# Sewer56/dxt-lossless-transform

Measured on AMD Instinct MI355X. Metric: GiB/s BC blocks transformed (fwd+inv), higher is better.
Workload: dtype u8

## Files before the change

dxt-lossless-transform_amd/_build.py:

```python
from __future__ import annotations

import hashlib
import os
import shutil
import subprocess
from concurrent.futures import ThreadPoolExecutor

_HERE = os.path.dirname(os.path.abspath(__file__))
CSRC = os.path.join(_HERE, "csrc")
LIB_PATH = os.path.join(_HERE, "libdxtlt_gfx950.so")
_BUILD_DIR = os.path.join(os.path.dirname(_HERE), "build")

SOURCES = ["bcn_kernels.hip", "batch_kernels.hip", "dxtlt_api.cpp", "host_staging.cpp", "host_sharded.cpp", "c_api_core.cpp", "c_api_stable.cpp", "auto_transform.cpp", "file_format.cpp",
           "bc7_kernels.hip", "bc7_api.cpp", "bc6h_kernels.hip", "bc6h_api.cpp", "granule_launch.cpp", "granule_host.cpp", "bc1_normalize.hip", "normalize_api.cpp", "batch_api.cpp", "bc23_normalize.hip",
           "normalize23_api.cpp", "color565_ops.hip", "color565_api.cpp", "bcn_decode.hip", "decode_api.cpp",
           "auto_kernels.hip", "numa_affinity.cpp", "estimate_kernels.hip", "estimate_api.cpp", "batch_auto_kernels.hip", "batch_auto_api.cpp", "pixel_kernels.hip", "pixels_api.cpp",
           "image_kernels.hip", "image_regions_kernels.hip", "image_api.cpp", "image_batch_kernels.hip", "image_batch_api.cpp",
           "bc7_image_kernels.hip", "bc7_image_regions_kernels.hip", "bc7_image_api.cpp",
           "bc7_image_batch_kernels.hip", "bc7_image_batch_api.cpp",
           "bc6h_image_kernels.hip", "bc6h_image_regions_kernels.hip", "bc6h_image_api.cpp"]
BASE_FLAGS = ["--offload-arch=gfx950", "-O3", "-std=c++17", "-fPIC", "-Wall", "-Wextra", "-Wno-unused-command-line-argument"]


def _extra_flags(extra_flags=None) -> list:
    return list(extra_flags or [])


def _dirs(extra: list):
    if not extra:
        return os.path.join(_BUILD_DIR, "obj"), LIB_PATH
    tag = hashlib.sha256(" ".join(extra).encode()).hexdigest()[:12]
    side = os.path.join(_BUILD_DIR, "side-" + tag)
    return os.path.join(side, "obj"), os.path.join(side, "libdxtlt_gfx950.so")


def _hipcc() -> str:
    for cand in (os.environ.get("HIPCC"), shutil.which("hipcc"), "/opt/rocm/bin/hipcc"):
        if cand and os.path.exists(cand):
            return cand
    raise RuntimeError("hipcc not found: libdxtlt_gfx950.so cannot be built (set HIPCC)")


def _sources():
    return [os.path.join(CSRC, s) for s in SOURCES if os.path.exists(os.path.join(CSRC, s))]


def _headers():
    inc = os.path.join(os.path.dirname(_HERE), "include")
    files = [os.path.join(CSRC, f) for f in os.listdir(CSRC) if f.endswith(".h")]
    if os.path.isdir(inc):
        files += [os.path.join(inc, f) for f in os.listdir(inc) if f.endswith(".h")]
    return files


def is_stale() -> bool:
    if not os.path.exists(LIB_PATH):
        return True
    t = os.path.getmtime(LIB_PATH)
    return any(os.path.getmtime(f) > t for f in _sources() + _headers())


def build(force: bool = False, verbose: bool = False, extra_flags=None) -> str:
    extra = _extra_flags(extra_flags)
    obj_dir, lib_path = _dirs(extra)
    if not extra and not force and not is_stale():
        return LIB_PATH
    hipcc = _hipcc()
    os.makedirs(obj_dir, exist_ok=True)
    flags = BASE_FLAGS + extra
    newest_header = max((os.path.getmtime(h) for h in _headers()), default=0.0)

    def obj(src: str) -> str:
        return os.path.join(obj_dir, os.path.basename(src) + ".o")

    todo = []
    for src in _sources():
        o = obj(src)
        if force or not os.path.exists(o) or os.path.getmtime(o) < max(os.path.getmtime(src), newest_header):
            todo.append(src)

    def compile_one(src: str) -> None:
        cmd = [hipcc] + flags + ["-x", "hip", "-c", src, "-o", obj(src) + ".tmp"]
        if verbose:
            print(" ".join(cmd))
        subprocess.check_call(cmd)
        os.replace(obj(src) + ".tmp", obj(src))

    with ThreadPoolExecutor(max_workers=min(8, os.cpu_count() or 1)) as pool:
        list(pool.map(compile_one, todo))
    if not todo and os.path.exists(lib_path) and all(os.path.getmtime(obj(s)) <= os.path.getmtime(lib_path) for s in _sources()):
        return lib_path
    cmd = [hipcc, "--offload-arch=gfx950", "-shared", "-fPIC"] + [obj(s) for s in _sources()] + ["-o", lib_path + ".tmp", "-lpthread"]
    if verbose:
        print(" ".join(cmd))
    subprocess.check_call(cmd)
    os.replace(lib_path + ".tmp", lib_path)
    return lib_path


if __name__ == "__main__":
    print(build(force=True, verbose=True))
```

dxt-lossless-transform_amd/csrc/batch_api.cpp:

```cpp
#include <hip/hip_runtime_api.h>

#include <algorithm>
#include <condition_variable>
#include <cstdlib>
#include <cstring>
#include <exception>
#include <mutex>
#include <thread>
#include <vector>

#include "../../include/dxtlt_gfx950.h"
#include "bcn_launch.h"
#include "granule_launch.h"
#include "host_common.h"
#include "table_ring.h"

namespace {

using namespace dxtlt_host;
using dxtlt::BatchEntry;

inline uint32_t item_block_bytes(uint8_t format)
{
    return is_pixel_format(format) ? (uint32_t)pixel_bytes_of(format) : format == 1 || format == 4 ? 8u : 16u;
}

const char* const kDeviceFormatText = "batch item: format must be 1..5 (BC1..BC5), 6 (BC6H) or 7 (BC7; 6 and 7 are this build's own formats; "
                                      "pixel formats 8 and 9 go through dxtlt_transform_batch_host or the calls of dxtlt_pixels.h)";
const char* const kHostFormatText = "batch item: format must be 1..5 (BC1..BC5), 6 (BC6H), 7 (BC7), 8 (4-byte pixels) or 9 (3-byte pixels; "
                                    "6 to 9 are this build's own formats)";

inline bool pixel_item_overlaps(const DxtltBatchItem& it)
{
    if (!is_pixel_format(it.format) || it.len == 0)
        return false;
    const uintptr_t a = reinterpret_cast<uintptr_t>(it.d_input), b = reinterpret_cast<uintptr_t>(it.d_output);
    return a < b + it.len && b < a + it.len;
}

int32_t launch_pixel_item(const DxtltBatchItem& it, void* stream)
{
    const uint64_t pixels = it.len / item_block_bytes(it.format);
    return pixel_device_range(pixel_bytes_of(it.format), it.inverse != 0, it.d_input, it.d_output, pixels, 0, pixels,
                              pixel_decorrelate_of(it.decorrelation_mode),
                              pixel_layout_of(it.split_alpha_endpoints != 0, it.split_colour_endpoints != 0), stream);
}

thread_local dxtlt_host::TableRing g_ring;

const bool kTableByCopyEngine = dxtlt::experiment_env("DXTLT_BATCH_TABLE_COPY") != nullptr && dxtlt::experiment_env("DXTLT_BATCH_TABLE_COPY")[0] == '1';

}

dxtlt_host::TableRing& dxtlt_host::thread_table_ring() { return g_ring; }

hipError_t dxtlt_host::upload_table(TableSlot* slot, size_t bytes, hipStream_t stream)
{
    if (kTableByCopyEngine)
        return hipMemcpyAsync(slot->dev, slot->host, bytes, hipMemcpyHostToDevice, stream);
    return dxtlt::launch_table_upload(slot->host_mapped, slot->dev, bytes, stream);
}

namespace {

int32_t batch_device(const DxtltBatchItem* items, size_t count, void* hip_stream, bool pixels_allowed)
{
    if (count == 0)
        return kOk;
    if (items == nullptr)
        return fail(kInvalidArgument, "NULL item array with count > 0");
    for (size_t i = 0; i < count; ++i) {
        const DxtltBatchItem& it = items[i];
        if (it.format < 1 || it.format > (pixels_allowed ? 9 : 7))
            return fail(kInvalidArgument, kDeviceFormatText);
        if (it.len % item_block_bytes(it.format) != 0)
            return fail(kInvalidLength, "batch item: len is not a multiple of the block size");
        if (it.decorrelation_mode > 3 && dxtlt::format_has_colour(it.format))
            return fail(kInvalidArgument, "batch item: decorrelation_mode must be 0..3");
        if (it.len > 0 && (it.d_input == nullptr || it.d_output == nullptr))
            return fail(kInvalidArgument, "batch item: NULL device buffer with len > 0");
        if (pixel_item_overlaps(it))
            return fail(kInvalidArgument, "batch item: pixel input and output overlap");
    }
    for (const int format : {7, 6}) {
        uint64_t granules[2] = {0, 0};
        for (size_t i = 0; i < count; ++i)
            if (items[i].format == format)
                granules[items[i].inverse ? 1 : 0] += items[i].len / 16 / 1024;
        if (granules[0] > 0xFFFFFFull || granules[1] > 0xFFFFFFull)
            return fail(kInvalidArgument, dxtlt::granule::named(format, "batch too large for one launch (256 GiB or more of ", " in one direction)"));
    }
    hipStream_t user = static_cast<hipStream_t>(hip_stream);

    struct Group {
        std::vector<BatchEntry> entries;
        uint32_t wgs = 0;
        uint32_t uniform_wgs = 0;
        bool uniform = true;
    };
    constexpr int kGroups = 5 * 2 * 16;
    std::vector<Group> groups(kGroups);
    auto group_settings = [](int gi) {
        dxtlt::Settings s{};
        s.variant = (gi >> 2) & 3;
        s.split_alpha = ((gi >> 1) & 1) != 0;
        s.split_colour = (gi & 1) != 0;
        return s;
    };
    std::vector<size_t> singles;
    for (size_t i = 0; i < count; ++i) {
        const DxtltBatchItem& it = items[i];
        if (it.len == 0 || dxtlt::granule::is_granule_format(it.format) || is_pixel_format(it.format))
            continue;
        if (it.len >= (size_t(64) << 30))
            return fail(kInvalidArgument, "batch item of 64 GiB or more: use the single-buffer entry point");
        const bool colour = dxtlt::format_has_colour(it.format);
        const int sa = dxtlt::format_has_alpha_split(it.format) && it.split_alpha_endpoints ? 1 : 0;
        const int sc = colour && it.split_colour_endpoints ? 1 : 0, mode = colour ? it.decorrelation_mode : 0;
        const int gi = (((it.format - 1) * 2 + (it.inverse ? 1 : 0)) << 4) | (mode << 2) | (sa << 1) | sc;
        Group& g = groups[gi];
        BatchEntry e{};
        e.src = static_cast<const uint8_t*>(it.d_input);
        e.dst = static_cast<uint8_t*>(it.d_output);
        e.blocks = it.len / item_block_bytes(it.format);
        e.first_wg = g.wgs;
        const uint32_t wgs = dxtlt::plan_batch_entry((dxtlt::Format)it.format, it.inverse != 0, group_settings(gi), e);
        if (wgs == 0xFFFFFFFFu) {
            singles.push_back(i);
            continue;
        }
        if ((uint64_t)g.wgs + wgs > 0xFFFFFFull)
            return fail(kInvalidArgument, "batch too large for one launch (64 GiB or more of one format, direction and settings)");
        g.wgs += wgs;
        g.entries.push_back(e);
        if (g.entries.size() == 1)
            g.uniform_wgs = wgs;
        else if (wgs != g.uniform_wgs)
            g.uniform = false;
    }
    static const bool no_uniform = dxtlt::experiment_env("DXTLT_BATCH_NO_UNIFORM") != nullptr;
    static const bool no_strided = dxtlt::experiment_env("DXTLT_BATCH_NO_STRIDED") != nullptr;

    using GranuleEntry = dxtlt::granule::BatchEntry;
    struct GranulePlan {
        std::vector<GranuleEntry> entries, tails;
        std::vector<uint32_t> coarse;
        uint64_t wgs = 0;
        size_t at = 0, entry_bytes = 0, tail_bytes = 0, bytes = 0;
    };
    GranulePlan granule_plans[4];
    size_t table_bytes = 0;
    for (int q = 0; q < 4; ++q) {
        GranulePlan& p = granule_plans[q];
        const int inverse = q & 1, format = q < 2 ? 7 : 6;
        for (size_t i = 0; i < count; ++i) {
            const DxtltBatchItem& it = items[i];
            if (it.format != format || it.len == 0 || (it.inverse != 0) != (inverse != 0))
                continue;
            const uint64_t blocks = it.len / 16, tail = blocks % 1024, main = blocks - tail;
            const uint8_t* src = static_cast<const uint8_t*>(it.d_input);
            uint8_t* dst = static_cast<uint8_t*>(it.d_output);
            if (main != 0) {
                p.entries.push_back({src, dst, main, (uint32_t)p.wgs, 0});
                p.wgs += main / 1024;
            }
            if (tail != 0)
                p.tails.push_back({src + main * 16, dst + main * 16, 0, 0, (uint32_t)tail});
        }
        if (p.entries.empty() && p.tails.empty())
            continue;
        p.coarse.resize(((size_t)p.wgs + 63) / 64);
        size_t cur = 0;
        for (size_t k = 0; k < p.coarse.size(); ++k) {
            while (cur + 1 < p.entries.size() && p.entries[cur + 1].first_wg <= (uint32_t)(k * 64))
                ++cur;
            p.coarse[k] = (uint32_t)cur;
        }
        p.entry_bytes = p.entries.size() * sizeof(GranuleEntry);
        p.tail_bytes = p.tails.size() * sizeof(GranuleEntry);
        p.bytes = (p.entry_bytes + p.tail_bytes + p.coarse.size() * sizeof(uint32_t) + 15) & ~(size_t)15;
        p.at = table_bytes;
        table_bytes += p.bytes;
    }

    struct Placed {
        int gi;
        size_t at, entry_bytes;
    };
    std::vector<Placed> placed;
    for (int gi = 0; gi < kGroups; ++gi) {
        const Group& g = groups[gi];
        if (g.entries.empty())
            continue;
        const size_t entry_bytes = (g.entries.size() * sizeof(BatchEntry) + 15) & ~(size_t)15;
        placed.push_back({gi, table_bytes, entry_bytes});
        table_bytes += entry_bytes + dxtlt::batch_index_bytes(g.wgs);
    }
    if (table_bytes != 0) {
        TableSlot* slot = nullptr;
        hipError_t e = g_ring.acquire(table_bytes, &slot);
        if (e != hipSuccess)
            return fail(kDevice, "batch table staging", e);
        for (const GranulePlan& p : granule_plans) {
            if (p.bytes == 0)
                continue;
            uint8_t* h = static_cast<uint8_t*>(slot->host) + p.at;
            if (p.entry_bytes) std::memcpy(h, p.entries.data(), p.entry_bytes);
            if (p.tail_bytes) std::memcpy(h + p.entry_bytes, p.tails.data(), p.tail_bytes);
            if (!p.coarse.empty()) std::memcpy(h + p.entry_bytes + p.tail_bytes, p.coarse.data(), p.coarse.size() * sizeof(uint32_t));
        }
        std::vector<bool> wide(placed.size());
        for (size_t k = 0; k < placed.size(); ++k) {
            const Group& g = groups[placed[k].gi];
            uint8_t* h = static_cast<uint8_t*>(slot->host) + placed[k].at;
            std::memcpy(h, g.entries.data(), g.entries.size() * sizeof(BatchEntry));
            wide[k] = dxtlt::build_batch_index(g.entries.data(), g.entries.size(), g.wgs, h + placed[k].entry_bytes);
        }
        e = upload_table(slot, table_bytes, user);
        const char* what = "batch table copy / launch";
        for (int q = 0; q < 4 && e == hipSuccess; ++q) {
            const GranulePlan& p = granule_plans[q];
            const int inverse = q & 1, format = q < 2 ? 7 : 6;
            if (p.bytes == 0)
                continue;
            const uint8_t* d = static_cast<const uint8_t*>(slot->dev) + p.at;
            e = dxtlt::granule::launch_batch(format, inverse != 0, reinterpret_cast<const GranuleEntry*>(d),
                                             reinterpret_cast<const uint32_t*>(d + p.entry_bytes + p.tail_bytes), (uint32_t)p.entries.size(),
                                             (uint32_t)p.wgs, reinterpret_cast<const GranuleEntry*>(d + p.entry_bytes),
                                             (uint32_t)p.tails.size(), user);
            if (e != hipSuccess)
                what = format == 7 ? "BC7 batch table copy / launch" : "BC6H batch table copy / launch";
        }
        for (size_t k = 0; k < placed.size() && e == hipSuccess; ++k) {
            const int gi = placed[k].gi;
            Group& g = groups[gi];
            const size_t n = g.entries.size();
            const bool uniform = g.uniform && !no_uniform;
            bool strided = uniform && !no_strided;
            const int64_t src_stride = n >= 2 ? (int64_t)(g.entries[1].src - g.entries[0].src) : 0;
            const int64_t dst_stride = n >= 2 ? (int64_t)(g.entries[1].dst - g.entries[0].dst) : 0;
            for (size_t i = 1; i < n && strided; ++i) {
                const BatchEntry &a = g.entries[0], &b = g.entries[i];
                strided = b.blocks == a.blocks && b.full_tiles == a.full_tiles && b.form == a.form && b.halo_vecs == a.halo_vecs &&
                          std::memcmp(b.shift, a.shift, sizeof a.shift) == 0 && std::memcmp(b.gbase, a.gbase, sizeof a.gbase) == 0 &&
                          b.src == a.src + (int64_t)i * src_stride && b.dst == a.dst + (int64_t)i * dst_stride;
            }
            const uint8_t* d = static_cast<const uint8_t*>(slot->dev) + placed[k].at;
            e = dxtlt::launch_batch((dxtlt::Format)((gi >> 5) + 1), ((gi >> 4) & 1) != 0, group_settings(gi),
                                    reinterpret_cast<const BatchEntry*>(d), d + placed[k].entry_bytes, (uint32_t)n, g.wgs,
                                    uniform ? g.uniform_wgs : 0, wide[k], user, strided ? &g.entries[0] : nullptr, src_stride, dst_stride);
        }
        hipError_t ev = hipEventRecord(slot->done, user);
        slot->pending = ev == hipSuccess;
        if (e != hipSuccess)
            return fail(kDevice, what, e);
        if (ev != hipSuccess)
            return fail(kDevice, "batch event", ev);
    }
    for (size_t i : singles) {
        const DxtltBatchItem& it = items[i];
        dxtlt::Settings s{};
        s.variant = it.decorrelation_mode;
        s.split_alpha = it.split_alpha_endpoints != 0;
        s.split_colour = it.split_colour_endpoints != 0;
        s = dxtlt::effective_settings((dxtlt::Format)it.format, s);
        const uint64_t blocks = it.len / item_block_bytes(it.format);
        const hipError_t e = dxtlt::launch_transform((dxtlt::Format)it.format, it.inverse != 0, s, it.d_input, it.d_output,
                                                     dxtlt::Range{blocks, 0, blocks}, user);
        if (e != hipSuccess)
            return fail(kDevice, "batch item launch", e);
    }
    for (size_t i = 0; i < count; ++i)
        if (is_pixel_format(items[i].format) && items[i].len != 0)
            if (int32_t rc = launch_pixel_item(items[i], user); rc != kOk)
                return rc;
    return kOk;
}

}

extern "C" int32_t dxtlt_transform_batch_device(const DxtltBatchItem* items, size_t count, void* hip_stream)
{
    return batch_device(items, count, hip_stream, false);
}

extern "C" uint32_t dxtlt_debug_plan_batch(int32_t format, int32_t inverse, int32_t variant, int32_t split_alpha, int32_t split_colour,
                                           const uint64_t* src_addresses, const uint64_t* dst_addresses, const uint64_t* blocks, size_t count,
                                           DxtltDebugPlannedEntry* entries_out, uint8_t* index_out, size_t index_capacity,
                                           uint32_t* index_is_wide_out)
{
    if (index_is_wide_out)
        *index_is_wide_out = 0;
    if (format < 1 || format > 5 || (count != 0 && (!src_addresses || !dst_addresses || !blocks || !entries_out)))
        return 0xFFFFFFFFu;
    dxtlt::Settings s{};
    s.variant = variant;
    s.split_alpha = split_alpha != 0;
    s.split_colour = split_colour != 0;
    s = dxtlt::effective_settings((dxtlt::Format)format, s);
    std::vector<BatchEntry> entries;
    uint32_t total = 0;
    for (size_t i = 0; i < count; ++i) {
        BatchEntry e{};
        e.src = reinterpret_cast<const uint8_t*>(static_cast<uintptr_t>(src_addresses[i]));
        e.dst = reinterpret_cast<uint8_t*>(static_cast<uintptr_t>(dst_addresses[i]));
        e.blocks = blocks[i];
        e.first_wg = total;
        const uint32_t wgs = dxtlt::plan_batch_entry((dxtlt::Format)format, inverse != 0, s, e);
        if (wgs == 0xFFFFFFFFu || (uint64_t)total + wgs > 0xFFFFFFull)
            return 0xFFFFFFFFu;
        if (wgs == 0)
            e.end_wg = e.first_wg;
        total += wgs;
        DxtltDebugPlannedEntry& o = entries_out[i];
        o.first_wg = e.first_wg;
        o.end_wg = e.end_wg;
        o.full_tiles = e.full_tiles;
        o.form = e.form;
        o.halo_vecs = e.halo_vecs;
        std::memcpy(o.shift, e.shift, sizeof o.shift);
        std::memcpy(o.gbase, e.gbase, sizeof o.gbase);
        if (wgs != 0)
            entries.push_back(e);
    }
    if (total != 0) {
        if (index_out == nullptr || index_capacity < dxtlt::batch_index_bytes(total))
            return 0xFFFFFFFFu;
        const bool wide = dxtlt::build_batch_index(entries.data(), entries.size(), total, index_out);
        if (index_is_wide_out)
            *index_is_wide_out = wide ? 1 : 0;
    }
    return total;
}

namespace {

size_t env_number(const char* name, size_t fallback)
{
    const char* v = std::getenv(name);
    const unsigned long long x = v ? std::strtoull(v, nullptr, 10) : 0;
    return x ? (size_t)x : fallback;
}
const size_t kHostBatchChunkBytes = env_number("DXTLT_BATCH_CHUNK_MIB", 64) << 20;
const int kCopyThreads = (int)std::min<size_t>(64, env_number("DXTLT_BATCH_THREADS", 6));

struct PinnedArenas {
    void* in[2] = {nullptr, nullptr};
    void* out[2] = {nullptr, nullptr};
    size_t cap = 0;
    ~PinnedArenas() { release(); }
    void release()
    {
        for (int i = 0; i < 2; ++i) {
            if (in[i]) (void)hipHostFree(in[i]);
            if (out[i]) (void)hipHostFree(out[i]);
            in[i] = out[i] = nullptr;
        }
        cap = 0;
    }
    hipError_t reserve(size_t bytes)
    {
        if (bytes <= cap)
            return hipSuccess;
        release();
        for (int i = 0; i < 2; ++i) {
            hipError_t e = hipHostMalloc(&in[i], bytes, hipHostMallocDefault);
            if (e == hipSuccess)
                e = hipHostMalloc(&out[i], bytes, hipHostMallocDefault);
            if (e != hipSuccess) {
                release();
                return e;
            }
        }
        cap = bytes;
        return hipSuccess;
    }
};
thread_local PinnedArenas g_pinned;
#define g_pinned_in(c) (pinned_in[(c) & 1])
#define g_pinned_out(c) (pinned_out[(c) & 1])

struct HostBatchShared {
    std::mutex m;
    std::condition_variable cv;
    std::vector<int> packed;
    std::vector<int> unpacked;
    int uploaded_recorded = 0;
    int kernels_issued = 0;
    int enqueued = 0;
    bool failed = false;
    hipError_t error = hipSuccess;
};

}

void dxtlt_host::release_batch_thread_tables()
{
    g_ring.release();
    g_pinned.release();
}

extern "C" int32_t dxtlt_transform_batch_host(const DxtltBatchItem* items, size_t count)
{
    if (count == 0)
        return kOk;
    if (items == nullptr)
        return fail(kInvalidArgument, "NULL item array with count > 0");
    uint64_t total = 0;
    for (size_t i = 0; i < count; ++i) {
        const DxtltBatchItem& it = items[i];
        if (it.format < 1 || it.format > 9)
            return fail(kInvalidArgument, kHostFormatText);
        if (it.len % item_block_bytes(it.format) != 0)
            return fail(kInvalidLength, "batch item: len is not a multiple of the block size");
        if (it.decorrelation_mode > 3 && dxtlt::format_has_colour(it.format))
            return fail(kInvalidArgument, "batch item: decorrelation_mode must be 0..3");
        if (it.len > 0 && (it.d_input == nullptr || it.d_output == nullptr))
            return fail(kInvalidArgument, "batch item: NULL buffer with len > 0");
        if (pixel_item_overlaps(it))
            return fail(kInvalidArgument, "batch item: pixel input and output overlap");
        if (it.len >= (size_t(4) << 30))
            return fail(kInvalidArgument, "batch item of 4 GiB or more: use the single-buffer entry point");
        total += (it.len + 255) & ~uint64_t(255);
    }
    if (total == 0)
        return kOk;

    const uint64_t big_item = 2 * (uint64_t)kHostBatchChunkBytes;
    std::vector<DxtltBatchItem> small;
    small.reserve(count);
    for (size_t i = 0; i < count; ++i) {
        const DxtltBatchItem& it = items[i];
        if (it.len < big_item) {
            small.push_back(it);
            continue;
        }
        int32_t rc;
        if (is_pixel_format(it.format))
            rc = pixel_host_call(pixel_bytes_of(it.format), it.inverse != 0, static_cast<const uint8_t*>(it.d_input),
                                 static_cast<uint8_t*>(it.d_output), it.len, pixel_decorrelate_of(it.decorrelation_mode),
                                 pixel_layout_of(it.split_alpha_endpoints != 0, it.split_colour_endpoints != 0));
        else if (dxtlt::granule::is_granule_format(it.format))
            rc = dxtlt_host::granule_host_call(it.format, it.inverse != 0, static_cast<const uint8_t*>(it.d_input),
                                               static_cast<uint8_t*>(it.d_output), it.len);
        else
            rc = dxtlt_host::transform(it.format, it.inverse != 0, static_cast<const uint8_t*>(it.d_input),
                                       static_cast<uint8_t*>(it.d_output), it.len, it.decorrelation_mode,
                                       dxtlt::format_has_alpha_split(it.format) && it.split_alpha_endpoints, it.split_colour_endpoints != 0);
        if (rc != kOk)
            return rc;
    }
    if (small.empty())
        return kOk;
    items = small.data();
    count = small.size();

    std::vector<uint64_t> slot(count);
    std::vector<size_t> chunk_first;
    std::vector<uint64_t> chunk_bytes;
    {
        uint64_t in_chunk = 0;
        chunk_first.push_back(0);
        for (size_t i = 0; i < count; ++i) {
            const uint64_t padded = (items[i].len + 255) & ~uint64_t(255);
            if (in_chunk > 0 && in_chunk + padded > kHostBatchChunkBytes) {
                chunk_first.push_back(i);
                chunk_bytes.push_back(in_chunk);
                in_chunk = 0;
            }
            slot[i] = in_chunk;
            in_chunk += padded;
        }
        chunk_first.push_back(count);
        chunk_bytes.push_back(in_chunk);
    }
    const int nchunks = (int)chunk_bytes.size();
    const uint64_t arena_bytes = *std::max_element(chunk_bytes.begin(), chunk_bytes.end());

    void *d_in = nullptr, *d_out = nullptr;
    hipStream_t up = nullptr;
    if (int32_t rc = acquire_staging((size_t)(2 * arena_bytes), &d_in, &d_out, &up); rc != kOk)
        return rc;
    if (hipError_t e = g_pinned.reserve((size_t)arena_bytes); e != hipSuccess)
        return fail(kDevice, "hipHostMalloc(batch arenas)", e);
    void* const pinned_in[2] = {g_pinned.in[0], g_pinned.in[1]};
    void* const pinned_out[2] = {g_pinned.out[0], g_pinned.out[1]};
    int dev = 0;
    (void)hipGetDevice(&dev);
    hipStream_t down = nullptr;
    if (hipError_t e = hipStreamCreateWithFlags(&down, hipStreamNonBlocking); e != hipSuccess)
        return fail(kDevice, "hipStreamCreate(download)", e);

    std::vector<hipEvent_t> ev((size_t)nchunks * 3, nullptr);
    for (auto& e : ev)
        if (hipError_t err = hipEventCreateWithFlags(&e, hipEventDisableTiming); err != hipSuccess) {
            for (auto& e2 : ev) if (e2) (void)hipEventDestroy(e2);
            (void)hipStreamDestroy(down);
            return fail(kDevice, "hipEventCreate", err);
        }
    auto ev_uploaded = [&](int c) { return ev[(size_t)c * 3]; };
    auto ev_kernels = [&](int c) { return ev[(size_t)c * 3 + 1]; };
    auto ev_downloaded = [&](int c) { return ev[(size_t)c * 3 + 2]; };

    HostBatchShared sh;
    sh.packed.assign((size_t)nchunks, 0);
    sh.unpacked.assign((size_t)nchunks, 0);
    auto set_failed = [&](hipError_t e) {
        std::lock_guard<std::mutex> lk(sh.m);
        if (!sh.failed) {
            sh.failed = true;
            sh.error = e;
        }
        sh.cv.notify_all();
    };

    auto packer = [&](int tid) {
        hipError_t e = hipSetDevice(dev);
        for (int c = 0; c < nchunks && e == hipSuccess; ++c) {
            if (c < 2) {
                std::lock_guard<std::mutex> lk(sh.m);
                if (sh.failed)
                    return;
            }
            if (c >= 2) {
                {
                    std::unique_lock<std::mutex> lk(sh.m);
                    sh.cv.wait(lk, [&] { return sh.uploaded_recorded > c - 2 || sh.failed; });
                    if (sh.failed)
                        return;
                }
                e = hipEventSynchronize(ev_uploaded(c - 2));
                if (e != hipSuccess)
                    break;
            }
            uint8_t* arena = static_cast<uint8_t*>(g_pinned_in(c));
            for (size_t i = chunk_first[(size_t)c] + (size_t)tid; i < chunk_first[(size_t)c + 1]; i += kCopyThreads)
                if (items[i].len)
                    std::memcpy(arena + slot[i], items[i].d_input, items[i].len);
            {
                std::lock_guard<std::mutex> lk(sh.m);
                sh.packed[(size_t)c]++;
            }
            sh.cv.notify_all();
        }
        if (e != hipSuccess)
            set_failed(e);
    };
    auto unpacker = [&](int tid) {
        hipError_t e = hipSetDevice(dev);
        for (int c = 0; c < nchunks && e == hipSuccess; ++c) {
            {
                std::unique_lock<std::mutex> lk(sh.m);
                sh.cv.wait(lk, [&] { return sh.enqueued > c || sh.failed; });
                if (sh.enqueued <= c)
                    return;
            }
            e = hipEventSynchronize(ev_downloaded(c));
            if (e != hipSuccess)
                break;
            const uint8_t* arena = static_cast<const uint8_t*>(g_pinned_out(c));
            for (size_t i = chunk_first[(size_t)c] + (size_t)tid; i < chunk_first[(size_t)c + 1]; i += kCopyThreads)
                if (items[i].len)
                    std::memcpy(items[i].d_output, arena + slot[i], items[i].len);
            {
                std::lock_guard<std::mutex> lk(sh.m);
                sh.unpacked[(size_t)c]++;
            }
            sh.cv.notify_all();
        }
        if (e != hipSuccess)
            set_failed(e);
    };

    std::vector<std::thread> threads;
    bool spawn_failed = false;
    auto spawn = [&](auto&& fn, auto... args) {
        if (spawn_failed)
            return;
        try {
            threads.emplace_back(fn, args...);
        } catch (const std::exception&) {
            spawn_failed = true;
        }
    };
    for (int t = 0; t < kCopyThreads; ++t) spawn(packer, t);
    for (int t = 0; t < kCopyThreads; ++t) spawn(unpacker, t);

    auto downloader = [&] {
        hipError_t e = hipSetDevice(dev);
        for (int c = 0; c < nchunks && e == hipSuccess; ++c) {
            {
                std::unique_lock<std::mutex> lk(sh.m);
                sh.cv.wait(lk, [&] { return (sh.kernels_issued > c && (c < 2 || sh.unpacked[(size_t)c - 2] == kCopyThreads)) || sh.failed; });
                if (sh.failed)
                    return;
            }
            const uint8_t* dout = static_cast<const uint8_t*>(d_out) + (size_t)(c & 1) * arena_bytes;
            e = hipStreamWaitEvent(down, ev_kernels(c), 0);
            if (e == hipSuccess)
                e = hipMemcpyAsync(g_pinned_out(c), dout, (size_t)chunk_bytes[(size_t)c], hipMemcpyDeviceToHost, down);
            if (e == hipSuccess)
                e = hipEventRecord(ev_downloaded(c), down);
            if (e != hipSuccess)
                break;
            {
                std::lock_guard<std::mutex> lk(sh.m);
                sh.enqueued = c + 1;
            }
            sh.cv.notify_all();
        }
        if (e != hipSuccess)
            set_failed(e);
    };
    spawn(downloader);
    if (spawn_failed) {
        set_failed(hipErrorOutOfMemory);
        for (auto& t : threads)
            t.join();
        for (auto& e : ev) (void)hipEventDestroy(e);
        (void)hipStreamDestroy(down);
        return fail(kAllocation, "could not start the batch copy threads");
    }

    int32_t rc = kOk;
    hipError_t err = hipSuccess;
    std::vector<DxtltBatchItem> dev_items;
    for (int c = 0; c < nchunks && rc == kOk && err == hipSuccess; ++c) {
        {
            std::unique_lock<std::mutex> lk(sh.m);
            sh.cv.wait(lk, [&] { return (sh.packed[(size_t)c] == kCopyThreads && (c < 2 || sh.enqueued > c - 2)) || sh.failed; });
            if (sh.failed)
                break;
        }
        uint8_t* di = static_cast<uint8_t*>(d_in) + (size_t)(c & 1) * arena_bytes;
        uint8_t* dout = static_cast<uint8_t*>(d_out) + (size_t)(c & 1) * arena_bytes;
        if (c >= 2)
            err = hipStreamWaitEvent(up, ev_kernels(c - 2), 0);
        if (err == hipSuccess)
            err = hipMemcpyAsync(di, g_pinned_in(c), (size_t)chunk_bytes[(size_t)c], hipMemcpyHostToDevice, up);
        if (err == hipSuccess)
            err = hipEventRecord(ev_uploaded(c), up);
        {
            std::lock_guard<std::mutex> lk(sh.m);
            if (err == hipSuccess)
                sh.uploaded_recorded = c + 1;
        }
        sh.cv.notify_all();
        if (err != hipSuccess)
            break;
        if (c >= 2)
            err = hipStreamWaitEvent(up, ev_downloaded(c - 2), 0);
        if (err != hipSuccess)
            break;
        dev_items.clear();
        for (size_t i = chunk_first[(size_t)c]; i < chunk_first[(size_t)c + 1]; ++i) {
            DxtltBatchItem it = items[i];
            it.d_input = di + slot[i];
            it.d_output = dout + slot[i];
            dev_items.push_back(it);
        }
        rc = batch_device(dev_items.data(), dev_items.size(), up, true);
        if (rc != kOk)
            break;
        err = hipEventRecord(ev_kernels(c), up);
        if (err != hipSuccess)
            break;
        {
            std::lock_guard<std::mutex> lk(sh.m);
            sh.kernels_issued = c + 1;
        }
        sh.cv.notify_all();
    }
    if (rc != kOk || err != hipSuccess) {
        std::lock_guard<std::mutex> lk(sh.m);
        sh.failed = true;
        if (err != hipSuccess && sh.error == hipSuccess)
            sh.error = err;
        sh.cv.notify_all();
    }
    for (auto& t : threads)
        t.join();
    (void)hipStreamSynchronize(up);
    (void)hipStreamSynchronize(down);
    for (auto& e : ev) (void)hipEventDestroy(e);
    (void)hipStreamDestroy(down);
    if (rc != kOk)
        return rc;
    if (sh.failed)
        return fail(kDevice, "host batch copy", sh.error);
    return kOk;
}
```

dxt-lossless-transform_amd/csrc/batch_kernels.hip:

```cpp
#include <cstdlib>
#include <cstring>
#include <vector>

#include "bcn_device.h"

#include "batch_lookup.h"

namespace dxtlt {

struct BatchView {
    const uint8_t* src;
    uint8_t* dst;
    uint64_t blocks;
    uint32_t first_wg, end_wg, full_tiles;
    uint32_t flags;
    uint32_t shifts[2];
    uint64_t gbase[6];
};

__device__ __forceinline__ BatchView load_batch_entry(const BatchEntry* entry)
{
    const uint64_t* q = reinterpret_cast<const uint64_t*>(entry);
    const uint32_t* w = reinterpret_cast<const uint32_t*>(entry);
    BatchView v;
    v.src = (const uint8_t*)(global_cptr)q[0];
    v.dst = (uint8_t*)(global_ptr)q[1];
    v.blocks = q[2];
    v.first_wg = w[6];
    v.end_wg = w[7];
    v.full_tiles = w[8];
    v.flags = w[9];
    v.shifts[0] = w[10];
    v.shifts[1] = w[11];
#pragma unroll
    for (int i = 0; i < 6; ++i)
        v.gbase[i] = q[6 + i];
    return v;
}
__device__ __forceinline__ void pin_batch_view(BatchView& v)
{
#ifdef DXTLT_WG_TIMING
    (void)v;
    return;
#endif
    uint64_t s = reinterpret_cast<uintptr_t>(v.src), d = reinterpret_cast<uintptr_t>(v.dst);
    asm("" : "+s"(s), "+s"(d), "+s"(v.blocks));
    v.src = (const uint8_t*)(global_cptr)s;
    v.dst = (uint8_t*)(global_ptr)d;
    asm("" : "+s"(v.first_wg), "+s"(v.end_wg), "+s"(v.full_tiles), "+s"(v.flags), "+s"(v.shifts[0]), "+s"(v.shifts[1]));
#pragma unroll
    for (int i = 0; i < 6; ++i)
        asm("" : "+s"(v.gbase[i]));
}
static_assert(offsetof(BatchEntry, first_wg) == 24 && offsetof(BatchEntry, end_wg) == 28 && offsetof(BatchEntry, full_tiles) == 32 && offsetof(BatchEntry, form) == 36 &&
                  offsetof(BatchEntry, shift) == 40 && offsetof(BatchEntry, gbase) == 48,
              "load_batch_entry reads BatchEntry by dword offsets");

constexpr uint32_t kBatchAligned = 1;

struct StridedBatch {
    BatchEntry first;
    int64_t src_stride, dst_stride;
    uint32_t on;
};

#ifdef DXTLT_WG_TIMING
__device__ uint32_t g_wg_timing[4 << 20];
extern "C" int dxtlt_debug_read_wg_timing(uint32_t* out, size_t count)
{
    return (int)hipMemcpyFromSymbol(out, HIP_SYMBOL(g_wg_timing), count * 4);
}
extern "C" int dxtlt_debug_read_wg_marks(uint32_t* out, size_t count)
{
    return (int)hipMemcpyFromSymbol(out, HIP_SYMBOL(dxtlt::g_wg_marks), count * 4);
}
#define WG_TIMING_BEGIN const uint64_t t_begin = __builtin_amdgcn_s_memrealtime();
#define WG_TIMING_END(kind)                                                                         \
    do {                                                                                            \
        __builtin_amdgcn_s_waitcnt(0);                                                              \
        asm volatile("s_waitcnt vmcnt(0)" ::: "memory");                                            \
        if (threadIdx.x == 0 && blockIdx.x < (1u << 20)) {                                          \
            uint32_t xcc;                                                                           \
            asm volatile("s_getreg_b32 %0, hwreg(HW_REG_XCC_ID)" : "=s"(xcc));                       \
            g_wg_timing[4 * blockIdx.x] = (uint32_t)(__builtin_amdgcn_s_memrealtime() - t_begin);   \
            g_wg_timing[4 * blockIdx.x + 1] = (kind);                                               \
            g_wg_timing[4 * blockIdx.x + 2] = (uint32_t)t_begin;                                    \
            g_wg_timing[4 * blockIdx.x + 3] = xcc & 0xF;                                            \
        }                                                                                           \
    } while (0)
#else
#define WG_TIMING_BEGIN
#define WG_TIMING_END(kind)
#endif

template <int FMT, int VARIANT, bool SA, bool SC, bool INVERSE, int THREADS = batch_tile_threads(FMT, SC, INVERSE)>
__global__ void __launch_bounds__(THREADS)
batch_kernel(const BatchEntry* __restrict__ entries_arg, const uint8_t* __restrict__ index_arg, uint32_t n_base, uint32_t uniform_wgs,
             uint32_t magic, StridedBatch strided)
{
    constexpr int kLds = INVERSE ? shift_lds_bytes(1, THREADS) : halo_lds_bytes<FMT, THREADS>();
    __shared__ __attribute__((aligned(16))) uint8_t lds[kLds];
    const uint32_t wg = blockIdx.x;
    WG_TIMING_BEGIN
    BatchView en;
    uint32_t e;
    uint64_t entries_at = reinterpret_cast<uintptr_t>(entries_arg), index_at = reinterpret_cast<uintptr_t>(index_arg);
#ifndef DXTLT_WG_TIMING
    asm("" : "+s"(entries_at), "+s"(index_at), "+s"(n_base), "+s"(uniform_wgs), "+s"(magic));
#endif
    const BatchEntry* entries = (const BatchEntry*)(const __attribute__((address_space(1))) BatchEntry*)entries_at;
    const uint8_t* index = (const uint8_t*)(global_cptr)index_at;
    if (uniform_wgs != 0) {
        e = __umulhi(wg, magic);
        if ((e + 1) * uniform_wgs <= wg)
            ++e;
        if (strided.on != 0) {
            const BatchEntry& f = strided.first;
            en.src = (const uint8_t*)(global_cptr)(reinterpret_cast<uintptr_t>(f.src) + (uint64_t)((int64_t)e * strided.src_stride));
            en.dst = (uint8_t*)(global_ptr)(reinterpret_cast<uintptr_t>(f.dst) + (uint64_t)((int64_t)e * strided.dst_stride));
            en.blocks = f.blocks;
            en.first_wg = e * uniform_wgs;
            en.end_wg = en.first_wg + uniform_wgs;
            en.full_tiles = f.full_tiles;
            en.flags = (uint32_t)f.form | ((uint32_t)f.halo_vecs << 8) | ((uint32_t)f.natural << 16);
            en.shifts[0] = (uint32_t)f.shift[0] | ((uint32_t)f.shift[1] << 8) | ((uint32_t)f.shift[2] << 16) | ((uint32_t)f.shift[3] << 24);
            en.shifts[1] = (uint32_t)f.shift[4] | ((uint32_t)f.shift[5] << 8);
#pragma unroll
            for (int i = 0; i < 6; ++i)
                en.gbase[i] = f.gbase[i];
        } else {
            en = load_batch_entry(entries + e);
        }
    } else {
        e = batch_entry_of_workgroup(entries, index, n_base, magic, wg, en);
    }
    const uint32_t n_wgs = en.end_wg - en.first_wg;
    uint32_t local = wg - en.first_wg;
    if (n_wgs >= 8) {
        local += (en.first_wg + n_wgs - 1u - e) & 7u;
        local = local >= n_wgs ? local - n_wgs : local;
    }
    const bool aligned = (en.flags & 0xFF) == kBatchAligned;
    if (aligned && local < en.full_tiles) {
        if constexpr (INVERSE)
            inv_aligned_tile<FMT, VARIANT, SA, SC, THREADS>(en.src, en.dst, en.blocks, 0, local, lds);
        else
            fwd_aligned_tile<FMT, VARIANT, SA, SC, THREADS>(en.src, en.dst, en.blocks, 0, local, lds);
        WG_TIMING_END(1);
        return;
    }
    Shifts sh;
#pragma unroll
    for (int i = 0; i < 6; ++i) {
        sh.d[i] = (int)((en.shifts[i >> 2] >> (8 * (i & 3))) & 127u);
        sh.gbase[i] = en.gbase[i];
    }
#ifdef DXTLT_EXPERIMENTS
    sh.xcd_remap = 0;
    sh.line_policy = INVERSE ? 1 : 3;
    sh.skip_partial = 0;
#endif
    sh.natural = 1;
    sh.halo_vecs = (int)(en.flags >> 8) & 0xFF;
    sh.full_tiles = en.full_tiles;
    sh.range_blocks = en.blocks;
    if constexpr (INVERSE) {
        if (local < en.full_tiles) {
            const uint64_t tile = xcd_contiguous_tile(local, en.full_tiles);
            inv_shift_tile<FMT, VARIANT, SA, SC, THREADS>(en.src, en.dst, en.blocks, 0, sh, tile, lds);
            WG_TIMING_END(2);
            return;
        }
        inv_shift_edge_tile<FMT, VARIANT, SA, SC, THREADS>(en.src, en.dst, en.blocks, sh, en.full_tiles, lds);
        WG_TIMING_END(4);
    } else {
        if (local != 0 && local < en.full_tiles) {
            fwd_halo_tile<FMT, VARIANT, SA, SC, kNormNone, true, THREADS>(en.src, en.dst, en.blocks, 0, sh, local, lds);
            WG_TIMING_END(2);
            return;
        }
        fwd_halo_edge_tile<FMT, VARIANT, SA, SC, kNormNone, true, THREADS>(en.src, en.dst, sh, local, lds);
        WG_TIMING_END(local == 0 ? 3 : 4);
    }
}

uint32_t plan_batch_entry(Format fmt, bool inverse, const Settings& s, BatchEntry& e)
{
    if (e.blocks == 0)
        return 0;
    const Settings es = effective_settings(fmt, s);
    const Streams S = make_streams(fmt, es.split_alpha, es.split_colour);
    const void* soa = inverse ? (const void*)e.src : (const void*)e.dst;
    const uint64_t T = (uint64_t)tile_blocks(fmt, batch_tile_threads(fmt, es.split_colour, inverse));
    const uint64_t tiles = e.blocks / T, rest = e.blocks % T;
    const uint64_t mask = inverse ? 15 : (uint64_t)(kHaloAlign - 1);
    bool on_lines = true, stream_tails = false;
    int d[6] = {0, 0, 0, 0, 0, 0}, halo_blocks = 0;
    for (int i = 0; i < S.n; ++i) {
        const uint64_t base = reinterpret_cast<uintptr_t>(soa) + (uint64_t)S.off[i] * e.blocks;
        d[i] = (int)(base & mask);
        on_lines = on_lines && (base & 127) == 0;
        stream_tails = stream_tails || d[i] != 0;
        halo_blocks = std::max(halo_blocks, (d[i] + S.width[i] - 1) / S.width[i]);
    }
    if (!shifts_are_natural(S, d))
        return 0xFFFFFFFFu;
    e.form = on_lines ? 1 : 0;
    e.natural = 1;
    e.reserved = 0;
    e.reserved2[0] = e.reserved2[1] = 0;
    const int per_vec = 16 / fmt_block(fmt);
    e.halo_vecs = inverse ? 0 : (uint8_t)((halo_blocks + per_vec - 1) / per_vec);
    for (int i = 0; i < 6; ++i) {
        e.shift[i] = (uint8_t)d[i];
        e.gbase[i] = i < S.n ? (uint64_t)S.off[i] * e.blocks - (uint64_t)d[i] : 0;
    }
    e.full_tiles = (uint32_t)tiles;
    const bool edge = rest != 0 || (!inverse && stream_tails);
    const uint32_t wgs = (uint32_t)tiles + (edge ? 1u : 0u);
    e.end_wg = e.first_wg + wgs;
    return wgs;
}

bool build_batch_index(const BatchEntry* entries, size_t n_entries, uint32_t total_wgs, uint8_t* index)
{
    const size_t n_base = batch_index_base_count(total_wgs), n_delta = batch_index_delta_count(total_wgs);
    uint32_t* base = reinterpret_cast<uint32_t*>(index);
    std::memset(index, 0, batch_index_bytes(total_wgs));
    std::vector<uint32_t> d(n_delta);
    uint32_t largest = 0;
    size_t cur = 0;
    for (size_t j = 0; j < n_delta; ++j) {
        const uint32_t wg = (uint32_t)(j * kBatchIndexWgs);
        while (cur + 1 < n_entries && entries[cur].end_wg <= wg)
            ++cur;
        if (wg % kBatchBaseWgs == 0)
            base[wg / kBatchBaseWgs] = (uint32_t)cur;
        d[j] = (uint32_t)(cur - base[wg / kBatchBaseWgs]);
        largest = std::max(largest, d[j]);
    }
    const bool wide = largest > 255;
    uint8_t* delta = index + n_base * 4;
    for (size_t j = 0; j < n_delta; ++j) {
        if (wide) {
            delta[2 * j] = (uint8_t)d[j];
            delta[2 * j + 1] = (uint8_t)(d[j] >> 8);
        } else {
            delta[j] = (uint8_t)d[j];
        }
    }
    return wide;
}

namespace {

using BatchFn = void (*)(const BatchEntry*, const uint8_t*, uint32_t, uint32_t, uint32_t, StridedBatch);

template <int FMT, int VARIANT, bool SA, bool SC>
BatchFn batch_fn(bool inverse) { return inverse ? batch_kernel<FMT, VARIANT, SA, SC, true> : batch_kernel<FMT, VARIANT, SA, SC, false>; }

template <int FMT, int VARIANT>
BatchFn batch_splits(bool sa, bool sc, bool inverse)
{
    if constexpr (FMT == kBc3) {
        if (sa)
            return sc ? batch_fn<FMT, VARIANT, true, true>(inverse) : batch_fn<FMT, VARIANT, true, false>(inverse);
    }
    return sc ? batch_fn<FMT, VARIANT, false, true>(inverse) : batch_fn<FMT, VARIANT, false, false>(inverse);
}

template <int FMT>
BatchFn batch_bc45(bool split_endpoints, bool inverse)
{
    return split_endpoints ? batch_fn<FMT, kNone, true, false>(inverse) : batch_fn<FMT, kNone, false, false>(inverse);
}

template <int FMT>
BatchFn batch_variant(int variant, bool sa, bool sc, bool inverse)
{
    switch (variant) {
    case kNone: return batch_splits<FMT, kNone>(sa, sc, inverse);
    case kVar1: return batch_splits<FMT, kVar1>(sa, sc, inverse);
    case kVar2: return batch_splits<FMT, kVar2>(sa, sc, inverse);
    default: return batch_splits<FMT, kVar3>(sa, sc, inverse);
    }
}

}

hipError_t launch_batch(Format fmt, bool inverse, const Settings& s, const BatchEntry* d_entries, const uint8_t* d_index,
                        uint32_t n_entries, uint32_t total_wgs, uint32_t uniform_wgs, bool wide_index, hipStream_t stream,
                        const BatchEntry* strided_first, int64_t src_stride, int64_t dst_stride)
{
    if (n_entries == 0 || total_wgs == 0)
        return hipSuccess;
    if (s.variant < 0 || s.variant > 3 || total_wgs > 0xFFFFFFu)
        return hipErrorInvalidValue;
    if (uniform_wgs != 0 && (uint64_t)uniform_wgs * n_entries != total_wgs)
        return hipErrorInvalidValue;
    const uint32_t magic = uniform_wgs > 1 ? (uint32_t)((1ull << 32) / uniform_wgs) : uniform_wgs == 1 ? 0xFFFFFFFFu : n_entries;
    static const bool no_array = experiment_env("DXTLT_BATCH_NO_ARRAY") != nullptr;
    if (strided_first != nullptr && uniform_wgs != 0 && !no_array && strided_first->form == 1) {
        const hipError_t e = launch_tiled_array(fmt, inverse, s, strided_first->src, strided_first->dst, strided_first->blocks, n_entries,
                                                src_stride, dst_stride, stream);
        if (e != hipErrorNotSupported)
            return e;
    }
    StridedBatch strided{};
    if (strided_first != nullptr && uniform_wgs != 0) {
        strided.first = *strided_first;
        strided.src_stride = src_stride;
        strided.dst_stride = dst_stride;
        strided.on = 1;
    }
    const Settings es = effective_settings(fmt, s);
    const bool sa = es.split_alpha, sc = es.split_colour;
    BatchFn k = nullptr;
    switch (fmt) {
    case kBc1: k = batch_variant<kBc1>(es.variant, false, sc, inverse); break;
    case kBc2: k = batch_variant<kBc2>(es.variant, false, sc, inverse); break;
    case kBc3: k = batch_variant<kBc3>(es.variant, sa, sc, inverse); break;
    case kBc4: k = batch_bc45<kBc4>(sa, inverse); break;
    case kBc5: k = batch_bc45<kBc5>(sa, inverse); break;
    default: return hipErrorInvalidValue;
    }
    hipLaunchKernelGGL(k, dim3(total_wgs), dim3(batch_tile_threads(fmt, sc, inverse)), 0, stream, d_entries, d_index,
                       (uint32_t)batch_index_base_count(total_wgs) | (wide_index ? 0x80000000u : 0u), uniform_wgs, magic, strided);
    return hipGetLastError();
}

}
```

dxt-lossless-transform_amd/csrc/bcn_device.h:

```cpp
#pragma once
#include <hip/hip_runtime.h>

#include <algorithm>
#include <cstddef>
#include <type_traits>

#include "bc1_normalize.h"
#include "bcn_launch.h"
#include "streaming_store.h"
#include "ycocg_swar.h"

namespace dxtlt {

typedef uint32_t u32x4 __attribute__((ext_vector_type(4)));
typedef uint32_t u32x2 __attribute__((ext_vector_type(2)));

constexpr int kThreads = 256;
constexpr int default_tile_threads(int fmt, bool inverse)
{
    (void)inverse;
    return fmt == kBc1 || fmt == kBc4 ? 128 : 256;
}

#ifndef DXTLT_NONTEMPORAL
#define DXTLT_NONTEMPORAL 1
#endif

#ifdef DXTLT_WG_TIMING
__device__ uint32_t g_wg_marks[8 << 20];
__device__ __forceinline__ void wg_mark(int i)
{
    if (threadIdx.x == 0 && blockIdx.x < (1u << 20))
        g_wg_marks[8 * blockIdx.x + i] = (uint32_t)__builtin_amdgcn_s_memrealtime();
}
#define WG_MARK(i) wg_mark(i)
#define WG_MARK_LOADS_DONE(i)                                  \
    do {                                                       \
        asm volatile("s_waitcnt vmcnt(0)" ::: "memory");       \
        wg_mark(i);                                            \
    } while (0)
#else
#define WG_MARK(i)
#define WG_MARK_LOADS_DONE(i)
#endif

__device__ __forceinline__ u32x4 gload16(const void* p)
{
#if DXTLT_NONTEMPORAL
    return __builtin_nontemporal_load(reinterpret_cast<const u32x4*>(p));
#else
    return *reinterpret_cast<const u32x4*>(p);
#endif
}

__device__ __forceinline__ void gstore16(void* p, u32x4 v)
{
#if DXTLT_NONTEMPORAL
    store_streaming16(p, v);
#else
    *reinterpret_cast<u32x4*>(p) = v;
#endif
}

__device__ __forceinline__ void gstore16_aos(uint8_t* aos_base, void* p, u32x4 v)
{
    if ((reinterpret_cast<uintptr_t>(aos_base) & 15) == 0)
        gstore16(p, v);
    else
        __builtin_nontemporal_store(v, reinterpret_cast<u32x4*>(p));
}

template <int I, int N, typename F>
__device__ __forceinline__ void static_for(F&& f)
{
    if constexpr (I < N) {
        f(std::integral_constant<int, I>{});
        static_for<I + 1, N>(f);
    }
}

template <int W, int WAVES, typename F>
__device__ __forceinline__ void for_this_wave_from(int w, F&& f)
{
    if constexpr (W + 1 >= WAVES) {
        f(std::integral_constant<int, W>{});
    } else {
        if (w == W)
            f(std::integral_constant<int, W>{});
        else
            for_this_wave_from<W + 1, WAVES>(w, f);
    }
}
template <int WAVES, typename F>
__device__ __forceinline__ void for_this_wave(int t, F&& f)
{
    for_this_wave_from<0, WAVES>(__builtin_amdgcn_readfirstlane(t >> 6), f);
}

__host__ __device__ constexpr int fmt_block(int fmt) { return fmt == kBc1 || fmt == kBc4 ? 8 : 16; }
__host__ __device__ constexpr int tile_blocks(int fmt, int threads) { return threads * 16 / fmt_block(fmt); }

template <int FMT, bool SA, bool SC, int T>
__device__ __forceinline__ uint64_t soa_offset_of_image_byte(int o, uint64_t total_blocks, uint64_t blk0)
{
    constexpr Streams S = make_streams(FMT, SA, SC);
    uint64_t r = 0;
#pragma unroll
    for (int s = 0; s < S.n; ++s) {
        const int lo = S.off[s] * T;
        const int hi = lo + S.width[s] * T;
        if (o >= lo && o < hi)
            r = (uint64_t)S.off[s] * total_blocks + (uint64_t)S.width[s] * blk0 + (uint64_t)(o - lo);
    }
    return r;
}

#ifndef DXTLT_WAVE_OFFSETS
#define DXTLT_WAVE_OFFSETS 1
#endif
template <int FMT, bool SA, bool SC, int T, int W>
__device__ __forceinline__ uint64_t soa_offset_of_image_byte_in_wave(int o, uint64_t total_blocks, uint64_t blk0)
{
    constexpr Streams S = make_streams(FMT, SA, SC);
    constexpr int wave_lo = W * 1024, wave_hi = wave_lo + 1024;
    uint64_t r = 0;
    static_for<0, S.n>([&](auto si) {
        constexpr int s = decltype(si)::value;
        constexpr int lo = S.off[s] * T;
        constexpr int hi = lo + S.width[s] * T;
        if constexpr (lo < wave_hi && hi > wave_lo) {
            constexpr bool only = lo <= wave_lo && hi >= wave_hi;
            const uint64_t base = (uint64_t)S.off[s] * total_blocks + (uint64_t)S.width[s] * blk0;
            if (only || (o >= lo && o < hi))
                r = base + (uint64_t)(uint32_t)(o - lo);
        }
    });
    return r;
}

template <int FMT, bool SA, bool SC, int THREADS>
__device__ __forceinline__ uint64_t soa_offset_of_lane(int t, uint64_t total_blocks, uint64_t blk0)
{
    constexpr int T = tile_blocks(FMT, THREADS);
#if DXTLT_WAVE_OFFSETS
    uint64_t o = 0;
    for_this_wave<THREADS / 64>(t, [&](auto wi) {
        o = soa_offset_of_image_byte_in_wave<FMT, SA, SC, T, decltype(wi)::value>(t * 16, total_blocks, blk0);
    });
    return o;
#else
    return soa_offset_of_image_byte<FMT, SA, SC, T>(t * 16, total_blocks, blk0);
#endif
}

template <typename T>
__device__ __forceinline__ T& lds_at(uint8_t* lds, int byte_off)
{
    return *reinterpret_cast<T*>(lds + byte_off);
}

typedef volatile uint16_t __attribute__((address_space(3))) lds_halfword;
__device__ __forceinline__ lds_halfword* lds_halfwords(uint8_t* lds, int byte_off)
{
    return (lds_halfword*)(lds + byte_off);
}

#ifndef DXTLT_BC3_RECORD6
#define DXTLT_BC3_RECORD6 1
#endif
typedef uint32_t u32x2_align4 __attribute__((ext_vector_type(2), aligned(4)));
typedef volatile uint32_t __attribute__((address_space(3))) lds_dword;

__device__ __forceinline__ void lds_put_record6(uint8_t* lds, int addr, uint32_t lo16, uint32_t hi32)
{
#if DXTLT_BC3_RECORD6
    const bool odd = (addr & 2) != 0;
    const int a32 = odd ? addr + 2 : addr;
    const int a16 = odd ? addr : addr + 4;
    const uint32_t v32 = odd ? hi32 : (lo16 & 0xFFFFu) | (hi32 << 16);
    const uint32_t v16 = odd ? lo16 : hi32 >> 16;
    *(lds_dword*)(lds + a32) = v32;
    *lds_halfwords(lds, a16) = (uint16_t)v16;
#else
    lds_halfwords(lds, addr)[0] = (uint16_t)lo16;
    lds_halfwords(lds, addr)[1] = (uint16_t)hi32;
    lds_halfwords(lds, addr)[2] = (uint16_t)(hi32 >> 16);
#endif
}

__device__ __forceinline__ void lds_get_record6(uint8_t* lds, int addr, uint32_t& lo16, uint32_t& hi32)
{
#if DXTLT_BC3_RECORD6
    const u32x2_align4 w = *reinterpret_cast<const u32x2_align4*>(lds + (addr & ~3));
    const uint32_t sh = (uint32_t)(addr & 2) * 8u;
    const uint32_t rec = __builtin_amdgcn_alignbit(w.y, w.x, sh);
    lo16 = rec & 0xFFFFu;
    hi32 = (rec >> 16) | ((w.y >> sh) << 16);
#else
    lo16 = lds_at<uint16_t>(lds, addr + 0);
    hi32 = (uint32_t)lds_at<uint16_t>(lds, addr + 2) | ((uint32_t)lds_at<uint16_t>(lds, addr + 4) << 16);
#endif
}

template <bool SA, int T, int E>
__device__ __forceinline__ void scatter_bc4_half(uint8_t* lds, int b, uint32_t lo, uint32_t hi)
{
    if constexpr (SA) {
        lds_at<uint8_t>(lds, E * T + b) = (uint8_t)lo;
        lds_at<uint8_t>(lds, (E + 1) * T + b) = (uint8_t)(lo >> 8);
    } else {
        lds_at<uint16_t>(lds, E * T + 2 * b) = (uint16_t)lo;
    }
    lds_put_record6(lds, (E + 2) * T + 6 * b, lo >> 16, hi);
}

template <bool SA, int T, int E>
__device__ __forceinline__ void gather_bc4_half(uint8_t* lds, int b, uint32_t& lo, uint32_t& hi)
{
    uint32_t a01;
    if constexpr (SA)
        a01 = (uint32_t)lds_at<uint8_t>(lds, E * T + b) | ((uint32_t)lds_at<uint8_t>(lds, (E + 1) * T + b) << 8);
    else
        a01 = lds_at<uint16_t>(lds, E * T + 2 * b);
    uint32_t i01;
    lds_get_record6(lds, (E + 2) * T + 6 * b, i01, hi);
    lo = a01 | (i01 << 16);
}

template <int FMT, int VARIANT, bool SA, bool SC, int T>
__device__ __forceinline__ void scatter_to_image(uint8_t* lds, int u, u32x4 q)
{
    if constexpr (FMT == kBc4) {
        if constexpr (SA) {
            lds_at<uint16_t>(lds, 0 * T + 2 * u) = (uint16_t)((q.x & 0xFFu) | ((q.z & 0xFFu) << 8));
            lds_at<uint16_t>(lds, 1 * T + 2 * u) = (uint16_t)(((q.x >> 8) & 0xFFu) | (q.z & 0xFF00u));
        } else {
            lds_at<uint32_t>(lds, 0 * T + 4 * u) = (q.x & 0xFFFFu) | (q.z << 16);
        }
        lds_at<uint32_t>(lds, 2 * T + 12 * u + 0) = (q.x >> 16) | (q.y << 16);
        lds_at<uint32_t>(lds, 2 * T + 12 * u + 4) = (q.y >> 16) | (q.z & 0xFFFF0000u);
        lds_at<uint32_t>(lds, 2 * T + 12 * u + 8) = q.w;
    } else if constexpr (FMT == kBc5) {
        scatter_bc4_half<SA, T, 0>(lds, u, q.x, q.y);
        scatter_bc4_half<SA, T, 8>(lds, u, q.z, q.w);
    } else if constexpr (FMT == kBc1) {
        const uint32_t ca = decorrelate2<VARIANT>(q.x);
        const uint32_t cb = decorrelate2<VARIANT>(q.z);
        if constexpr (SC) {
            lds_at<uint32_t>(lds, 0 * T + 4 * u) = (ca & 0xFFFFu) | (cb << 16);
            lds_at<uint32_t>(lds, 2 * T + 4 * u) = (ca >> 16) | (cb & 0xFFFF0000u);
        } else {
            lds_at<u32x2>(lds, 0 * T + 8 * u) = u32x2{ca, cb};
        }
        lds_at<u32x2>(lds, 4 * T + 8 * u) = u32x2{q.y, q.w};
    } else if constexpr (FMT == kBc2) {
        const uint32_t c = decorrelate2<VARIANT>(q.z);
        lds_at<u32x2>(lds, 0 * T + 8 * u) = u32x2{q.x, q.y};
        if constexpr (SC) {
            lds_at<uint16_t>(lds, 8 * T + 2 * u) = (uint16_t)c;
            lds_at<uint16_t>(lds, 10 * T + 2 * u) = (uint16_t)(c >> 16);
        } else {
            lds_at<uint32_t>(lds, 8 * T + 4 * u) = c;
        }
        lds_at<uint32_t>(lds, 12 * T + 4 * u) = q.w;
    } else {
        const uint32_t c = decorrelate2<VARIANT>(q.z);
        if constexpr (SA) {
            lds_at<uint8_t>(lds, 0 * T + u) = (uint8_t)q.x;
            lds_at<uint8_t>(lds, 1 * T + u) = (uint8_t)(q.x >> 8);
        } else {
            lds_at<uint16_t>(lds, 0 * T + 2 * u) = (uint16_t)q.x;
        }
        lds_put_record6(lds, 2 * T + 6 * u, q.x >> 16, q.y);
        if constexpr (SC) {
            lds_at<uint16_t>(lds, 8 * T + 2 * u) = (uint16_t)c;
            lds_at<uint16_t>(lds, 10 * T + 2 * u) = (uint16_t)(c >> 16);
        } else {
            lds_at<uint32_t>(lds, 8 * T + 4 * u) = c;
        }
        lds_at<uint32_t>(lds, 12 * T + 4 * u) = q.w;
    }
}

template <int FMT, int VARIANT, bool SA, bool SC, int T>
__device__ __forceinline__ u32x4 gather_from_image(uint8_t* lds, int u)
{
    u32x4 q;
    if constexpr (FMT == kBc4) {
        uint32_t e;
        if constexpr (SA) {
            const uint32_t a0 = lds_at<uint16_t>(lds, 0 * T + 2 * u), a1 = lds_at<uint16_t>(lds, 1 * T + 2 * u);
            e = (a0 & 0xFFu) | ((a1 & 0xFFu) << 8) | ((a0 & 0xFF00u) << 8) | ((a1 & 0xFF00u) << 16);
        } else {
            e = lds_at<uint32_t>(lds, 0 * T + 4 * u);
        }
        const uint32_t r0 = lds_at<uint32_t>(lds, 2 * T + 12 * u + 0);
        const uint32_t r1 = lds_at<uint32_t>(lds, 2 * T + 12 * u + 4);
        const uint32_t r2 = lds_at<uint32_t>(lds, 2 * T + 12 * u + 8);
        q.x = (e & 0xFFFFu) | (r0 << 16);
        q.y = (r0 >> 16) | (r1 << 16);
        q.z = (e >> 16) | (r1 & 0xFFFF0000u);
        q.w = r2;
    } else if constexpr (FMT == kBc5) {
        uint32_t rlo, rhi, glo, ghi;
        gather_bc4_half<SA, T, 0>(lds, u, rlo, rhi);
        gather_bc4_half<SA, T, 8>(lds, u, glo, ghi);
        q = u32x4{rlo, rhi, glo, ghi};
    } else if constexpr (FMT == kBc1) {
        uint32_t ca, cb;
        if constexpr (SC) {
            const uint32_t c0 = lds_at<uint32_t>(lds, 0 * T + 4 * u);
            const uint32_t c1 = lds_at<uint32_t>(lds, 2 * T + 4 * u);
            ca = (c0 & 0xFFFFu) | (c1 << 16);
            cb = (c0 >> 16) | (c1 & 0xFFFF0000u);
        } else {
            const u32x2 p = lds_at<u32x2>(lds, 0 * T + 8 * u);
            ca = p.x;
            cb = p.y;
        }
        const u32x2 idx = lds_at<u32x2>(lds, 4 * T + 8 * u);
        q.x = recorrelate2<VARIANT>(ca);
        q.y = idx.x;
        q.z = recorrelate2<VARIANT>(cb);
        q.w = idx.y;
    } else if constexpr (FMT == kBc2) {
        const u32x2 a = lds_at<u32x2>(lds, 0 * T + 8 * u);
        uint32_t c;
        if constexpr (SC)
            c = (uint32_t)lds_at<uint16_t>(lds, 8 * T + 2 * u) | ((uint32_t)lds_at<uint16_t>(lds, 10 * T + 2 * u) << 16);
        else
            c = lds_at<uint32_t>(lds, 8 * T + 4 * u);
        q.x = a.x;
        q.y = a.y;
        q.z = recorrelate2<VARIANT>(c);
        q.w = lds_at<uint32_t>(lds, 12 * T + 4 * u);
    } else {
        uint32_t a01;
        if constexpr (SA)
            a01 = (uint32_t)lds_at<uint8_t>(lds, 0 * T + u) | ((uint32_t)lds_at<uint8_t>(lds, 1 * T + u) << 8);
        else
            a01 = lds_at<uint16_t>(lds, 0 * T + 2 * u);
        uint32_t i01, i2345;
        lds_get_record6(lds, 2 * T + 6 * u, i01, i2345);
        uint32_t c;
        if constexpr (SC)
            c = (uint32_t)lds_at<uint16_t>(lds, 8 * T + 2 * u) | ((uint32_t)lds_at<uint16_t>(lds, 10 * T + 2 * u) << 16);
        else
            c = lds_at<uint32_t>(lds, 8 * T + 4 * u);
        q.x = a01 | (i01 << 16);
        q.y = i2345;
        q.z = recorrelate2<VARIANT>(c);
        q.w = lds_at<uint32_t>(lds, 12 * T + 4 * u);
    }
    return q;
}

__device__ __forceinline__ uint64_t xcd_contiguous_tile(uint32_t orig, uint32_t nwg)
{
    const uint32_t q = nwg >> 3, r = nwg & 7, xcd = orig & 7;
    const uint32_t start = xcd < r ? xcd * (q + 1) : r * (q + 1) + (xcd - r) * q;
    return start + (orig >> 3);
}


template <int FMT, int NORM>
__device__ __forceinline__ u32x4 normalize_vector(u32x4 q)
{
    if constexpr (FMT == kBc1 && NORM != kNormNone) {
        uint32_t ca = q.x, xa = q.y, cb = q.z, xb = q.w;
        normalize_bc1_block<NORM>(ca, xa);
        normalize_bc1_block<NORM>(cb, xb);
        q = u32x4{ca, xa, cb, xb};
    }
    return q;
}

constexpr int kTiledArray = 2;

template <int FMT, int VARIANT, bool SA, bool SC, int THREADS, int NORM = kNormNone>
__device__ __forceinline__ void fwd_aligned_tile(const uint8_t* __restrict__ aos, uint8_t* __restrict__ soa,
                                                 uint64_t total_blocks, uint64_t first_block, uint64_t tile, uint8_t* lds)
{
    constexpr int T = tile_blocks(FMT, THREADS);
    const int t = threadIdx.x;
    WG_MARK(1);
    const u32x4 q = normalize_vector<FMT, NORM>(gload16(aos + tile * (THREADS * 16) + t * 16));
    WG_MARK_LOADS_DONE(2);
    scatter_to_image<FMT, VARIANT, SA, SC, T>(lds, t, q);
    __syncthreads();
    WG_MARK(3);
    const u32x4 v = lds_at<u32x4>(lds, t * 16);
    const uint64_t o = soa_offset_of_lane<FMT, SA, SC, THREADS>(t, total_blocks, first_block + tile * T);
    gstore16(soa + o, v);
    WG_MARK(4);
}

struct AosSink {
    template <int FMT, int THREADS>
    __device__ __forceinline__ void store(uint8_t* aos, uint64_t tile, int t, u32x4 q) const
    {
        gstore16_aos(aos, aos + tile * (THREADS * 16) + t * 16, q);
    }
    template <int FMT, int THREADS>
    __device__ __forceinline__ void store_edge(uint8_t* aos, uint64_t tile, int t, u32x4 q, int own) const
    {
        constexpr int PV = 16 / fmt_block(FMT);
        uint8_t* out = aos + tile * (THREADS * 16) + t * 16;
        if ((t + 1) * PV <= own)
            __builtin_nontemporal_store(q, reinterpret_cast<u32x4*>(out));
        else
            __builtin_nontemporal_store(u32x2{q.x, q.y}, reinterpret_cast<u32x2*>(out));
    }
};

template <int FMT, int VARIANT, bool SA, bool SC, int THREADS, typename SINK = AosSink>
__device__ __forceinline__ void inv_aligned_tile(const uint8_t* __restrict__ soa, uint8_t* __restrict__ aos,
                                                 uint64_t total_blocks, uint64_t first_block, uint64_t tile, uint8_t* lds,
                                                 const SINK& sink = SINK{})
{
    constexpr int T = tile_blocks(FMT, THREADS);
    const int t = threadIdx.x;
    const uint64_t o = soa_offset_of_lane<FMT, SA, SC, THREADS>(t, total_blocks, first_block + tile * T);
    lds_at<u32x4>(lds, t * 16) = gload16(soa + o);
    __syncthreads();
    const u32x4 q = gather_from_image<FMT, VARIANT, SA, SC, T>(lds, t);
    sink.template store<FMT, THREADS>(aos, tile, t, q);
}

template <int FMT, int VARIANT, bool SA, bool SC, int THREADS, int NORM = kNormNone>
__global__ void __launch_bounds__(THREADS)
fwd_tiled(const uint8_t* __restrict__ aos, uint8_t* __restrict__ soa, uint64_t total_blocks, uint64_t first_block,
          int xcd_remap, int64_t aos_stride, int64_t soa_stride)
{
    __shared__ __attribute__((aligned(16))) uint8_t lds[THREADS * 16];
    WG_MARK(0);
    if (xcd_remap & kTiledArray) {
        aos += (int64_t)blockIdx.y * aos_stride;
        soa += (int64_t)blockIdx.y * soa_stride;
    }
#ifdef DXTLT_EXPERIMENTS
    const uint64_t tile = (xcd_remap & 1) ? xcd_contiguous_tile(blockIdx.x, gridDim.x) : (uint64_t)blockIdx.x;
#else
    const uint64_t tile = blockIdx.x;
#endif
    fwd_aligned_tile<FMT, VARIANT, SA, SC, THREADS, NORM>(aos, soa, total_blocks, first_block, tile, lds);
}

template <int FMT, int VARIANT, bool SA, bool SC, int THREADS>
__global__ void __launch_bounds__(THREADS)
inv_tiled(const uint8_t* __restrict__ soa, uint8_t* __restrict__ aos, uint64_t total_blocks, uint64_t first_block,
          int xcd_remap, int64_t soa_stride, int64_t aos_stride)
{
    __shared__ __attribute__((aligned(16))) uint8_t lds[THREADS * 16];
    if (xcd_remap & kTiledArray) {
        soa += (int64_t)blockIdx.y * soa_stride;
        aos += (int64_t)blockIdx.y * aos_stride;
    }
#ifdef DXTLT_EXPERIMENTS
    const uint64_t tile = (xcd_remap & 1) ? xcd_contiguous_tile(blockIdx.x, gridDim.x) : (uint64_t)blockIdx.x;
#else
    const uint64_t tile = blockIdx.x;
#endif
    inv_aligned_tile<FMT, VARIANT, SA, SC, THREADS>(soa, aos, total_blocks, first_block, tile, lds);
}

struct Shifts {
    int d[6];
    int natural;
    int halo_vecs;
    uint64_t gbase[6];
    uint32_t full_tiles;
    uint64_t range_blocks;
#ifdef DXTLT_EXPERIMENTS
    int xcd_remap;
    int line_policy;
    int skip_partial;
#endif
};

__device__ __forceinline__ bool shifts_xcd_contiguous(const Shifts& sh, bool product_default)
{
#ifdef DXTLT_EXPERIMENTS
    (void)product_default;
    return sh.xcd_remap != 0;
#else
    (void)sh;
    return product_default;
#endif
}
__device__ __forceinline__ bool shifts_halo_write_through(const Shifts& sh)
{
#ifdef DXTLT_EXPERIMENTS
    return sh.line_policy == 3;
#else
    (void)sh;
    return true;
#endif
}
__device__ __forceinline__ bool shifts_skip_partial(const Shifts& sh)
{
#ifdef DXTLT_EXPERIMENTS
    return sh.skip_partial != 0;
#else
    (void)sh;
    return false;
#endif
}

template <typename STREAMS>
__host__ __device__ inline void fill_gbase(Shifts& sh, const STREAMS& S, uint64_t total_blocks, uint64_t first_block)
{
    for (int i = 0; i < 6; ++i)
        sh.gbase[i] = i < S.n ? (uint64_t)S.off[i] * total_blocks + (uint64_t)S.width[i] * first_block - (uint64_t)sh.d[i] : 0;
}

typedef const __attribute__((address_space(1))) uint8_t* global_cptr;
typedef __attribute__((address_space(1))) uint8_t* global_ptr;

__device__ __forceinline__ const uint8_t* fetched_now(const uint8_t* p)
{
    uint64_t v = reinterpret_cast<uintptr_t>(p);
    asm("" : "+s"(v));
    return (const uint8_t*)(global_cptr)v;
}
__device__ __forceinline__ uint8_t* fetched_now(uint8_t* p)
{
    uint64_t v = reinterpret_cast<uintptr_t>(p);
    asm("" : "+s"(v));
    return (uint8_t*)(global_ptr)v;
}

__device__ __forceinline__ Shifts shifts_fetched_at_once(const Shifts& in)
{
    Shifts s = in;
#ifdef DXTLT_EXPERIMENTS
    asm("" : "+s"(s.d[0]), "+s"(s.d[1]), "+s"(s.d[2]), "+s"(s.d[3]), "+s"(s.d[4]), "+s"(s.d[5]), "+s"(s.gbase[0]), "+s"(s.gbase[1]),
             "+s"(s.gbase[2]), "+s"(s.gbase[3]), "+s"(s.gbase[4]), "+s"(s.gbase[5]), "+s"(s.xcd_remap), "+s"(s.line_policy),
             "+s"(s.skip_partial), "+s"(s.natural), "+s"(s.halo_vecs), "+s"(s.full_tiles), "+s"(s.range_blocks));
#else
    asm("" : "+s"(s.d[0]), "+s"(s.d[1]), "+s"(s.d[2]), "+s"(s.d[3]), "+s"(s.d[4]), "+s"(s.d[5]), "+s"(s.gbase[0]), "+s"(s.gbase[1]),
             "+s"(s.gbase[2]), "+s"(s.gbase[3]), "+s"(s.gbase[4]), "+s"(s.gbase[5]), "+s"(s.natural), "+s"(s.halo_vecs),
             "+s"(s.full_tiles), "+s"(s.range_blocks));
#endif
    return s;
}

__host__ __device__ constexpr int stream_element_width(int bytes_per_block) { return bytes_per_block == 6 ? 2 : bytes_per_block; }

template <typename STREAMS>
__host__ __device__ inline int shifts_are_natural(const STREAMS& S, const int (&d)[6])
{
    int ok = 1;
    for (int i = 0; i < 6; ++i)
        if (i < S.n && (d[i] & (stream_element_width(S.width[i]) - 1)) != 0)
            ok = 0;
    return ok;
}


template <typename T>
using lds_volatile = volatile T __attribute__((address_space(3)));

template <int SIZE>
__device__ __forceinline__ void lds_put_piece(uint8_t* lds, int addr, uint64_t v)
{
    if constexpr (SIZE == 1) *(lds_volatile<uint8_t>*)(lds + addr) = (uint8_t)v;
    if constexpr (SIZE == 2) *(lds_volatile<uint16_t>*)(lds + addr) = (uint16_t)v;
    if constexpr (SIZE == 4) *(lds_volatile<uint32_t>*)(lds + addr) = (uint32_t)v;
    if constexpr (SIZE == 8) *(lds_volatile<uint64_t>*)(lds + addr) = v;
}

template <int SIZE>
__device__ __forceinline__ uint64_t lds_get_piece(uint8_t* lds, int addr)
{
    if constexpr (SIZE == 1) return *(lds_volatile<uint8_t>*)(lds + addr);
    if constexpr (SIZE == 2) return *(lds_volatile<uint16_t>*)(lds + addr);
    if constexpr (SIZE == 4) return *(lds_volatile<uint32_t>*)(lds + addr);
    if constexpr (SIZE == 8) return *(lds_volatile<uint64_t>*)(lds + addr);
    return 0;
}

constexpr int lds_piece_size(int W, int K, int P)
{
    const int a = K + P;
    int align = a == 0 ? W : (a & -a);
    if (align > W) align = W;
    int size = 1;
    while (size * 2 <= align && size * 2 <= W - P) size *= 2;
    return size;
}

template <int W, int K, int P = 0>
__device__ __forceinline__ void lds_put_seq(uint8_t* lds, int addr, uint64_t v)
{
    if constexpr (P < W) {
        constexpr int size = lds_piece_size(W, K, P);
        lds_put_piece<size>(lds, addr + P, v >> (8 * P));
        lds_put_seq<W, K, P + size>(lds, addr, v);
    }
}

template <int W, int K, int P = 0>
__device__ __forceinline__ uint64_t lds_get_seq(uint8_t* lds, int addr)
{
    if constexpr (P < W) {
        constexpr int size = lds_piece_size(W, K, P);
        return (lds_get_piece<size>(lds, addr + P) << (8 * P)) | lds_get_seq<W, K, P + size>(lds, addr);
    }
    return 0;
}

template <int W, bool NAT = false>
__device__ __forceinline__ void lds_put(uint8_t* lds, int addr, uint64_t v)
{
    if constexpr (W == 1 || NAT) {
        lds_put_piece<W>(lds, addr, v);
    } else {
        switch (addr & (W - 1)) {
        case 0: lds_put_seq<W, 0>(lds, addr, v); break;
        case 1: lds_put_seq<W, 1>(lds, addr, v); break;
        case 2: if constexpr (W > 2) lds_put_seq<W, 2>(lds, addr, v); break;
        case 3: if constexpr (W > 2) lds_put_seq<W, 3>(lds, addr, v); break;
        case 4: if constexpr (W > 4) lds_put_seq<W, 4>(lds, addr, v); break;
        case 5: if constexpr (W > 4) lds_put_seq<W, 5>(lds, addr, v); break;
        case 6: if constexpr (W > 4) lds_put_seq<W, 6>(lds, addr, v); break;
        default: if constexpr (W > 4) lds_put_seq<W, 7>(lds, addr, v); break;
        }
    }
}

template <int W, bool NAT = false>
__device__ __forceinline__ uint64_t lds_get(uint8_t* lds, int addr)
{
    if constexpr (W == 1 || NAT) {
        return lds_get_piece<W>(lds, addr);
    } else {
        switch (addr & (W - 1)) {
        case 0: return lds_get_seq<W, 0>(lds, addr);
        case 1: return lds_get_seq<W, 1>(lds, addr);
        case 2: if constexpr (W > 2) return lds_get_seq<W, 2>(lds, addr); break;
        case 3: if constexpr (W > 2) return lds_get_seq<W, 3>(lds, addr); break;
        case 4: if constexpr (W > 4) return lds_get_seq<W, 4>(lds, addr); break;
        case 5: if constexpr (W > 4) return lds_get_seq<W, 5>(lds, addr); break;
        case 6: if constexpr (W > 4) return lds_get_seq<W, 6>(lds, addr); break;
        default: if constexpr (W > 4) return lds_get_seq<W, 7>(lds, addr); break;
        }
        return 0;
    }
}

template <int FMT, bool SA, bool SC>
struct FieldStreams {
    static constexpr int alpha = 0;
    static constexpr int a1 = 1;
    static constexpr int aidx = SA ? 2 : 1;
    static constexpr int col = FMT == kBc1 ? 0 : FMT == kBc2 ? 1 : (SA ? 3 : 2);
    static constexpr int c1 = col + 1;
    static constexpr int idx = col + (SC ? 2 : 1);
    static constexpr int galpha = aidx + 1;
    static constexpr int ga1 = galpha + 1;
    static constexpr int gaidx = SA ? galpha + 2 : galpha + 1;
};

template <bool SA, bool NAT, int ALPHA, int A1, int AIDX>
__device__ __forceinline__ void scatter_shifted_bc4_block(uint8_t* lds, int b, uint32_t lo, uint32_t hi, const int (&base)[6])
{
    if constexpr (SA) {
        lds_put<1>(lds, base[ALPHA] + b, lo & 0xFF);
        lds_put<1>(lds, base[A1] + b, (lo >> 8) & 0xFF);
    } else {
        lds_put<2, NAT>(lds, base[ALPHA] + 2 * b, lo & 0xFFFF);
    }
    if constexpr (NAT && DXTLT_BC3_RECORD6) {
        lds_put_record6(lds, base[AIDX] + 6 * b, lo >> 16, hi);
    } else {
        lds_put<2, NAT>(lds, base[AIDX] + 6 * b + 0, lo >> 16);
        lds_put<2, NAT>(lds, base[AIDX] + 6 * b + 2, hi & 0xFFFF);
        lds_put<2, NAT>(lds, base[AIDX] + 6 * b + 4, hi >> 16);
    }
}

template <bool SA, bool NAT, int ALPHA, int A1, int AIDX>
__device__ __forceinline__ void gather_shifted_bc4_block(uint8_t* lds, int b, uint32_t& lo, uint32_t& hi, const int (&base)[6])
{
    uint32_t a01;
    if constexpr (SA)
        a01 = (uint32_t)lds_get<1>(lds, base[ALPHA] + b) | ((uint32_t)lds_get<1>(lds, base[A1] + b) << 8);
    else
        a01 = (uint32_t)lds_get<2, NAT>(lds, base[ALPHA] + 2 * b);
    if constexpr (NAT && DXTLT_BC3_RECORD6) {
        uint32_t i01;
        lds_get_record6(lds, base[AIDX] + 6 * b, i01, hi);
        lo = a01 | (i01 << 16);
    } else {
        const uint32_t i01 = (uint32_t)lds_get<2, NAT>(lds, base[AIDX] + 6 * b + 0);
        const uint32_t i23 = (uint32_t)lds_get<2, NAT>(lds, base[AIDX] + 6 * b + 2);
        const uint32_t i45 = (uint32_t)lds_get<2, NAT>(lds, base[AIDX] + 6 * b + 4);
        lo = a01 | (i01 << 16);
        hi = i23 | (i45 << 16);
    }
}

template <int FMT, int VARIANT, bool SA, bool SC, bool NAT>
__device__ __forceinline__ void scatter_shifted(uint8_t* lds, int u, u32x4 q, const int (&base)[6])
{
    using F = FieldStreams<FMT, SA, SC>;
    if constexpr (FMT == kBc4) {
        scatter_shifted_bc4_block<SA, NAT, F::alpha, F::a1, F::aidx>(lds, 2 * u, q.x, q.y, base);
        scatter_shifted_bc4_block<SA, NAT, F::alpha, F::a1, F::aidx>(lds, 2 * u + 1, q.z, q.w, base);
    } else if constexpr (FMT == kBc5) {
        scatter_shifted_bc4_block<SA, NAT, F::alpha, F::a1, F::aidx>(lds, u, q.x, q.y, base);
        scatter_shifted_bc4_block<SA, NAT, F::galpha, F::ga1, F::gaidx>(lds, u, q.z, q.w, base);
    } else if constexpr (FMT == kBc1) {
        const uint32_t ca = decorrelate2<VARIANT>(q.x);
        const uint32_t cb = decorrelate2<VARIANT>(q.z);
        if constexpr (NAT) {
            if constexpr (SC) {
                lds_put<2, true>(lds, base[F::col] + 4 * u, ca & 0xFFFFu);
                lds_put<2, true>(lds, base[F::col] + 4 * u + 2, cb & 0xFFFFu);
                lds_put<2, true>(lds, base[F::c1] + 4 * u, ca >> 16);
                lds_put<2, true>(lds, base[F::c1] + 4 * u + 2, cb >> 16);
            } else {
                lds_put<4, true>(lds, base[F::col] + 8 * u, ca);
                lds_put<4, true>(lds, base[F::col] + 8 * u + 4, cb);
            }
            lds_put<4, true>(lds, base[F::idx] + 8 * u, q.y);
            lds_put<4, true>(lds, base[F::idx] + 8 * u + 4, q.w);
        } else {
            if constexpr (SC) {
                lds_put<4>(lds, base[F::col] + 4 * u, (ca & 0xFFFFu) | (cb << 16));
                lds_put<4>(lds, base[F::c1] + 4 * u, (ca >> 16) | (cb & 0xFFFF0000u));
            } else {
                lds_put<8>(lds, base[F::col] + 8 * u, (uint64_t)ca | ((uint64_t)cb << 32));
            }
            lds_put<8>(lds, base[F::idx] + 8 * u, (uint64_t)q.y | ((uint64_t)q.w << 32));
        }
    } else {
        const uint32_t c = decorrelate2<VARIANT>(q.z);
        if constexpr (FMT == kBc2) {
            lds_put<8, NAT>(lds, base[F::alpha] + 8 * u, (uint64_t)q.x | ((uint64_t)q.y << 32));
        } else {
            if constexpr (SA) {
                lds_put<1>(lds, base[F::alpha] + u, q.x & 0xFF);
                lds_put<1>(lds, base[F::a1] + u, (q.x >> 8) & 0xFF);
            } else {
                lds_put<2, NAT>(lds, base[F::alpha] + 2 * u, q.x & 0xFFFF);
            }
            if constexpr (NAT && DXTLT_BC3_RECORD6) {
                lds_put_record6(lds, base[F::aidx] + 6 * u, q.x >> 16, q.y);
            } else {
                lds_put<2, NAT>(lds, base[F::aidx] + 6 * u + 0, q.x >> 16);
                lds_put<2, NAT>(lds, base[F::aidx] + 6 * u + 2, q.y & 0xFFFF);
                lds_put<2, NAT>(lds, base[F::aidx] + 6 * u + 4, q.y >> 16);
            }
        }
        if constexpr (SC) {
            lds_put<2, NAT>(lds, base[F::col] + 2 * u, c & 0xFFFF);
            lds_put<2, NAT>(lds, base[F::c1] + 2 * u, c >> 16);
        } else {
            lds_put<4, NAT>(lds, base[F::col] + 4 * u, c);
        }
        lds_put<4, NAT>(lds, base[F::idx] + 4 * u, q.w);
    }
}

template <int FMT, int VARIANT, bool SA, bool SC, bool NAT>
__device__ __forceinline__ u32x4 gather_shifted(uint8_t* lds, int u, const int (&base)[6])
{
    using F = FieldStreams<FMT, SA, SC>;
    u32x4 q;
    if constexpr (FMT == kBc4 || FMT == kBc5) {
        constexpr bool two = FMT == kBc4;
        uint32_t alo, ahi, blo, bhi;
        gather_shifted_bc4_block<SA, NAT, F::alpha, F::a1, F::aidx>(lds, two ? 2 * u : u, alo, ahi, base);
        if constexpr (two)
            gather_shifted_bc4_block<SA, NAT, F::alpha, F::a1, F::aidx>(lds, 2 * u + 1, blo, bhi, base);
        else
            gather_shifted_bc4_block<SA, NAT, F::galpha, F::ga1, F::gaidx>(lds, u, blo, bhi, base);
        q = u32x4{alo, ahi, blo, bhi};
    } else if constexpr (FMT == kBc1) {
        uint32_t ca, cb;
        uint64_t idx;
        if constexpr (NAT) {
            if constexpr (SC) {
                ca = (uint32_t)lds_get<2, true>(lds, base[F::col] + 4 * u) | ((uint32_t)lds_get<2, true>(lds, base[F::c1] + 4 * u) << 16);
                cb = (uint32_t)lds_get<2, true>(lds, base[F::col] + 4 * u + 2) |
                     ((uint32_t)lds_get<2, true>(lds, base[F::c1] + 4 * u + 2) << 16);
            } else {
                ca = (uint32_t)lds_get<4, true>(lds, base[F::col] + 8 * u);
                cb = (uint32_t)lds_get<4, true>(lds, base[F::col] + 8 * u + 4);
            }
            idx = lds_get<4, true>(lds, base[F::idx] + 8 * u) | (lds_get<4, true>(lds, base[F::idx] + 8 * u + 4) << 32);
        } else {
            if constexpr (SC) {
                const uint32_t c0 = (uint32_t)lds_get<4>(lds, base[F::col] + 4 * u);
                const uint32_t c1 = (uint32_t)lds_get<4>(lds, base[F::c1] + 4 * u);
                ca = (c0 & 0xFFFFu) | (c1 << 16);
                cb = (c0 >> 16) | (c1 & 0xFFFF0000u);
            } else {
                const uint64_t p = lds_get<8>(lds, base[F::col] + 8 * u);
                ca = (uint32_t)p;
                cb = (uint32_t)(p >> 32);
            }
            idx = lds_get<8>(lds, base[F::idx] + 8 * u);
        }
        q.x = recorrelate2<VARIANT>(ca);
        q.y = (uint32_t)idx;
        q.z = recorrelate2<VARIANT>(cb);
        q.w = (uint32_t)(idx >> 32);
    } else {
        if constexpr (FMT == kBc2) {
            const uint64_t a = lds_get<8, NAT>(lds, base[F::alpha] + 8 * u);
            q.x = (uint32_t)a;
            q.y = (uint32_t)(a >> 32);
        } else {
            uint32_t a01;
            if constexpr (SA)
                a01 = (uint32_t)lds_get<1>(lds, base[F::alpha] + u) | ((uint32_t)lds_get<1>(lds, base[F::a1] + u) << 8);
            else
                a01 = (uint32_t)lds_get<2, NAT>(lds, base[F::alpha] + 2 * u);
            if constexpr (NAT && DXTLT_BC3_RECORD6) {
                uint32_t i01, i2345;
                lds_get_record6(lds, base[F::aidx] + 6 * u, i01, i2345);
                q.x = a01 | (i01 << 16);
                q.y = i2345;
            } else {
                const uint32_t i01 = (uint32_t)lds_get<2, NAT>(lds, base[F::aidx] + 6 * u + 0);
                const uint32_t i23 = (uint32_t)lds_get<2, NAT>(lds, base[F::aidx] + 6 * u + 2);
                const uint32_t i45 = (uint32_t)lds_get<2, NAT>(lds, base[F::aidx] + 6 * u + 4);
                q.x = a01 | (i01 << 16);
                q.y = i23 | (i45 << 16);
            }
        }
        uint32_t c;
        if constexpr (SC)
            c = (uint32_t)lds_get<2, NAT>(lds, base[F::col] + 2 * u) | ((uint32_t)lds_get<2, NAT>(lds, base[F::c1] + 2 * u) << 16);
        else
            c = (uint32_t)lds_get<4, NAT>(lds, base[F::col] + 4 * u);
        q.z = recorrelate2<VARIANT>(c);
        q.w = (uint32_t)lds_get<4, NAT>(lds, base[F::idx] + 4 * u);
    }
    return q;
}

template <bool TO_GLOBAL>
__device__ __forceinline__ void copy_partial_segment(uint8_t* dst, const uint8_t* src, int lo, int hi)
{
    auto mv = [&](int p, int w) {
        if (w == 1) dst[p] = src[p];
        if (w == 2) *reinterpret_cast<uint16_t*>(dst + p) = *reinterpret_cast<const uint16_t*>(src + p);
        if (w == 4) *reinterpret_cast<uint32_t*>(dst + p) = *reinterpret_cast<const uint32_t*>(src + p);
        if (w == 8) *reinterpret_cast<u32x2*>(dst + p) = *reinterpret_cast<const u32x2*>(src + p);
    };
    if (hi == 16) {
        int p = lo;
        if (p & 1) { mv(p, 1); p += 1; }
        if (p & 2) { mv(p, 2); p += 2; }
        if (p & 4) { mv(p, 4); p += 4; }
        if (p & 8) { mv(p, 8); }
    } else {
        int p = 0;
        if (hi & 8) { mv(p, 8); p += 8; }
        if (hi & 4) { mv(p, 4); p += 4; }
        if (hi & 2) { mv(p, 2); p += 2; }
        if (hi & 1) { mv(p, 1); }
    }
}

__device__ __forceinline__ uint64_t uniform64(uint64_t v)
{
    return ((uint64_t)(uint32_t)__builtin_amdgcn_readfirstlane((int)(uint32_t)(v >> 32)) << 32) |
           (uint32_t)__builtin_amdgcn_readfirstlane((int)(uint32_t)v);
}

template <int FMT, bool SA, bool SC, int T>
__device__ __forceinline__ void slice_bases(uint64_t tile, const Shifts& sh, uint64_t (&gb)[6])
{
    constexpr Streams S = make_streams(FMT, SA, SC);
#pragma unroll
    for (int s = 0; s < 6; ++s)
        gb[s] = s < S.n ? uniform64(sh.gbase[s] + tile * (uint64_t)(S.width[s] * T)) : 0;
}

constexpr int shift_lds_bytes(int r, int threads = 256) { return r * threads * 16 + 16 * 6; }
constexpr int kShiftLdsBytes = shift_lds_bytes(1);

#ifndef DXTLT_BC1_SHIFT_THREADS
#define DXTLT_BC1_SHIFT_THREADS 256
#endif
__host__ __device__ constexpr int shift_tile_threads(int fmt) { return fmt == kBc1 ? DXTLT_BC1_SHIFT_THREADS : 256; }
__host__ __device__ constexpr int halo_tile_threads(int fmt, bool split_colour)
{
    return fmt == kBc1 && !split_colour ? 128 : shift_tile_threads(fmt);
}
#ifndef DXTLT_BATCH_BC1_NOSPLIT_FWD_THREADS
#define DXTLT_BATCH_BC1_NOSPLIT_FWD_THREADS 128
#endif
__host__ __device__ constexpr int batch_tile_threads(int fmt, bool split_colour, bool inverse)
{
    return !inverse && fmt == kBc1 && !split_colour ? DXTLT_BATCH_BC1_NOSPLIT_FWD_THREADS : shift_tile_threads(fmt);
}


#ifndef DXTLT_HALO_ALIGN
#define DXTLT_HALO_ALIGN 64
#endif
constexpr int kHaloAlign = DXTLT_HALO_ALIGN;
constexpr int kHaloBlocks = kHaloAlign;
constexpr int kHaloPad = kHaloAlign;
template <int FMT, int THREADS = 256>
constexpr int halo_lds_bytes() { return fmt_block(FMT) * (tile_blocks(FMT, THREADS) + kHaloBlocks) + kHaloPad * 6; }

__device__ __forceinline__ void copy_segment_bytes(uint8_t* dst, const uint8_t* src, int lo, int hi)
{
    int p = lo;
#pragma clang loop vectorize(disable) unroll(disable)
    while (p < hi) {
        const int left = hi - p;
        if ((p & 7) == 0 && left >= 8) {
            *reinterpret_cast<u32x2*>(dst + p) = *reinterpret_cast<const u32x2*>(src + p);
            p += 8;
        } else if ((p & 3) == 0 && left >= 4) {
            *reinterpret_cast<uint32_t*>(dst + p) = *reinterpret_cast<const uint32_t*>(src + p);
            p += 4;
        } else if ((p & 1) == 0 && left >= 2) {
            *reinterpret_cast<uint16_t*>(dst + p) = *reinterpret_cast<const uint16_t*>(src + p);
            p += 2;
        } else {
            dst[p] = src[p];
            p += 1;
        }
    }
}

template <int FMT, bool SA, bool SC, int W, bool EDGE = false, int THREADS = 256>
__device__ __forceinline__ void halo_copy_out_wave(uint8_t* __restrict__ soa, const uint8_t* lds, int t, const uint64_t (&gb)[6],
                                                   const Shifts& sh, const int (&vlo)[6], const int (&vhi)[6])
{
    constexpr Streams S = make_streams(FMT, SA, SC);
    constexpr int T = tile_blocks(FMT, THREADS);
    constexpr int H = kHaloBlocks;
    constexpr int wave_lo = W * 1024, wave_hi = wave_lo + 1024;
    const int o = t * 16;
    int la = 0, wo = 0, lo_s = 0, hi_s = 0;
    uint64_t g = 0;
    static_for<0, S.n>([&](auto si) {
        constexpr int s = decltype(si)::value;
        constexpr int lo = S.off[s] * T;
        constexpr int hi = lo + S.width[s] * T;
        if constexpr (lo < wave_hi && hi > wave_lo) {
            constexpr bool only = lo <= wave_lo && hi >= wave_hi;
            if (only || (o >= lo && o < hi)) {
                la = S.off[s] * (T + H) + kHaloPad * s + S.width[s] * H + (o - lo);
                g = gb[s] + (uint64_t)(o - lo);
                if constexpr (EDGE) {
                    wo = o - lo;
                    lo_s = vlo[s];
                    hi_s = vhi[s];
                }
            }
        }
    });
    if constexpr (EDGE) {
        const int lo = lo_s - wo > 0 ? lo_s - wo : 0;
        const int hi = hi_s - wo < 16 ? hi_s - wo : 16;
        if (hi <= lo)
            return;
        if (lo != 0 || hi != 16)
            copy_segment_bytes(soa + g, lds + la, lo, hi);
        else
            __builtin_nontemporal_store(lds_at<u32x4>(const_cast<uint8_t*>(lds), la), reinterpret_cast<u32x4*>(soa + g));
        return;
    }
    if (shifts_halo_write_through(sh))
        gstore16(soa + g, lds_at<u32x4>(const_cast<uint8_t*>(lds), la));
    else
        __builtin_nontemporal_store(lds_at<u32x4>(const_cast<uint8_t*>(lds), la), reinterpret_cast<u32x4*>(soa + g));
}

template <int FMT, int VARIANT, bool SA, bool SC, int NORM, bool NAT, int THREADS = 256>
__device__ __forceinline__ void fwd_halo_tile(const uint8_t* __restrict__ aos, uint8_t* __restrict__ soa,
                                              uint64_t , uint64_t , const Shifts& sh, uint64_t tile,
                                              uint8_t* lds)
{
    constexpr Streams S = make_streams(FMT, SA, SC);
    constexpr int T = tile_blocks(FMT, THREADS);
    constexpr int H = kHaloBlocks;
    constexpr int HV = H * fmt_block(FMT) / 16;
    const int t = threadIdx.x;
    int base[6];
#pragma unroll
    for (int s = 0; s < 6; ++s)
        base[s] = s < S.n ? S.off[s] * (T + H) + kHaloPad * s + sh.d[s] + S.width[s] * H : 0;

    const uint8_t* tile_aos = aos + tile * (THREADS * 16);
    WG_MARK(1);
    const u32x4 q = *reinterpret_cast<const u32x4*>(tile_aos + t * 16);
    const int hv = sh.halo_vecs;
    const bool has_halo = tile > 0 && t < hv && !shifts_skip_partial(sh);
    if (has_halo) {
        const u32x4 qh = *reinterpret_cast<const u32x4*>(tile_aos - hv * 16 + t * 16);
        scatter_shifted<FMT, VARIANT, SA, SC, NAT>(lds, t - hv, normalize_vector<FMT, NORM>(qh), base);
    }
    static_assert(HV <= THREADS, "the halo is loaded by the first lanes of the workgroup");
    WG_MARK_LOADS_DONE(2);
    scatter_shifted<FMT, VARIANT, SA, SC, NAT>(lds, t, normalize_vector<FMT, NORM>(q), base);
    __syncthreads();
    WG_MARK(3);

    uint64_t gb[6];
    slice_bases<FMT, SA, SC, T>(tile, sh, gb);
    const int none[6] = {0, 0, 0, 0, 0, 0};
    if constexpr (THREADS == 256) {
        switch (__builtin_amdgcn_readfirstlane(t >> 6)) {
        case 0: halo_copy_out_wave<FMT, SA, SC, 0>(soa, lds, t, gb, sh, none, none); break;
        case 1: halo_copy_out_wave<FMT, SA, SC, 1>(soa, lds, t, gb, sh, none, none); break;
        case 2: halo_copy_out_wave<FMT, SA, SC, 2>(soa, lds, t, gb, sh, none, none); break;
        default: halo_copy_out_wave<FMT, SA, SC, 3>(soa, lds, t, gb, sh, none, none); break;
        }
    } else {
        for_this_wave<THREADS / 64>(t, [&](auto wi) {
            halo_copy_out_wave<FMT, SA, SC, decltype(wi)::value, false, THREADS>(soa, lds, t, gb, sh, none, none);
        });
    }
    WG_MARK(4);
}

struct EdgeSlot {
    int s;
    int wo;
    int width;
    int d;
    int lds_base;
    uint64_t g;
};

template <int FMT, bool SA, bool SC, int T, int LA, int LB, int LC>
__device__ __forceinline__ EdgeSlot edge_slot_of_image_byte(int o, const Shifts& sh, const uint64_t (&gb)[6])
{
    constexpr Streams S = make_streams(FMT, SA, SC);
    EdgeSlot e{0, 0, 1, 0, 0, 0};
    static_for<0, S.n>([&](auto si) {
        constexpr int s = decltype(si)::value;
        constexpr int lo = S.off[s] * T, hi = lo + S.width[s] * T;
        if (o >= lo && o < hi) {
            e.s = s;
            e.wo = o - lo;
            e.width = S.width[s];
            e.d = sh.d[s];
            e.lds_base = S.off[s] * LA + LB * s + S.width[s] * LC;
            e.g = gb[s];
        }
    });
    return e;
}

template <int FMT, bool SA, bool SC, int T, int LA, int LB, int LC>
__device__ __forceinline__ EdgeSlot edge_slot_behind_window(int s_sel, int k, const Shifts& sh, const uint64_t (&gb)[6])
{
    constexpr Streams S = make_streams(FMT, SA, SC);
    EdgeSlot e{0, 0, 1, 0, 0, 0};
    static_for<0, S.n>([&](auto si) {
        constexpr int s = decltype(si)::value;
        if (s == s_sel) {
            e.s = s;
            e.wo = S.width[s] * T + 16 * k;
            e.width = S.width[s];
            e.d = sh.d[s];
            e.lds_base = S.off[s] * LA + LB * s + S.width[s] * LC;
            e.g = gb[s];
        }
    });
    return e;
}

template <int FMT, int VARIANT, bool SA, bool SC, int NORM, bool NAT, int THREADS = 256>
__device__ __forceinline__ void fwd_halo_edge_tile(const uint8_t* __restrict__ aos, uint8_t* __restrict__ soa, const Shifts& sh,
                                                   uint64_t tile, uint8_t* lds)
{
    constexpr Streams S = make_streams(FMT, SA, SC);
    constexpr int T = tile_blocks(FMT, THREADS);
    constexpr int H = kHaloBlocks;
    constexpr int PV = 16 / fmt_block(FMT);
    const int t = threadIdx.x;
    int base[6];
#pragma unroll
    for (int s = 0; s < 6; ++s)
        base[s] = s < S.n ? S.off[s] * (T + H) + kHaloPad * s + sh.d[s] + S.width[s] * H : 0;

    const uint64_t left = sh.range_blocks - tile * (uint64_t)T;
    const int own = left < (uint64_t)T ? (int)left : T;
    const uint8_t* tile_aos = aos + tile * (THREADS * 16);
    const int hv = sh.halo_vecs;
    const bool has_halo = tile > 0 && t < hv;
    const bool whole_vec = (t + 1) * PV <= own;
    const bool half_vec = PV == 2 && !whole_vec && t * PV < own;
    u32x4 q = {0u, 0u, 0u, 0u}, qh = {0u, 0u, 0u, 0u};
    if (whole_vec)
        q = *reinterpret_cast<const u32x4*>(tile_aos + t * 16);
    if (half_vec) {
        const u32x2 h = *reinterpret_cast<const u32x2*>(tile_aos + t * 16);
        q = u32x4{h.x, h.y, 0u, 0u};
    }
    if (has_halo)
        qh = *reinterpret_cast<const u32x4*>(tile_aos - hv * 16 + t * 16);
    if (has_halo)
        scatter_shifted<FMT, VARIANT, SA, SC, NAT>(lds, t - hv, normalize_vector<FMT, NORM>(qh), base);
    if (whole_vec || half_vec)
        scatter_shifted<FMT, VARIANT, SA, SC, NAT>(lds, t, normalize_vector<FMT, NORM>(q), base);
    __syncthreads();

    uint64_t gb[6];
    slice_bases<FMT, SA, SC, T>(tile, sh, gb);
    int vlo[6], vhi[6];
#pragma unroll
    for (int s = 0; s < 6; ++s) {
        const int d = s < S.n ? sh.d[s] : 0, w = s < S.n ? S.width[s] : 0;
        vlo[s] = tile == 0 ? d : 0;
        vhi[s] = own == T ? w * T : d + w * own;
    }
    if constexpr (THREADS == 256) {
        switch (__builtin_amdgcn_readfirstlane(t >> 6)) {
        case 0: halo_copy_out_wave<FMT, SA, SC, 0, true>(soa, lds, t, gb, sh, vlo, vhi); break;
        case 1: halo_copy_out_wave<FMT, SA, SC, 1, true>(soa, lds, t, gb, sh, vlo, vhi); break;
        case 2: halo_copy_out_wave<FMT, SA, SC, 2, true>(soa, lds, t, gb, sh, vlo, vhi); break;
        default: halo_copy_out_wave<FMT, SA, SC, 3, true>(soa, lds, t, gb, sh, vlo, vhi); break;
        }
    } else {
        for_this_wave<THREADS / 64>(t, [&](auto wi) {
            halo_copy_out_wave<FMT, SA, SC, decltype(wi)::value, true, THREADS>(soa, lds, t, gb, sh, vlo, vhi);
        });
    }
    constexpr int XS = kHaloAlign / 16;
    if (t < XS * S.n) {
        const EdgeSlot e = edge_slot_behind_window<FMT, SA, SC, T, T + H, kHaloPad, H>(t / XS, t % XS, sh, gb);
        int hi_s = 0;
#pragma unroll
        for (int s = 0; s < 6; ++s)
            hi_s = s == e.s ? vhi[s] : hi_s;
        const int hi = hi_s - e.wo < 16 ? hi_s - e.wo : 16;
        if (hi > 0) {
            uint8_t* la = lds + e.lds_base + e.wo;
            uint8_t* g = soa + e.g + (uint64_t)(int64_t)e.wo;
            if (hi != 16)
                copy_segment_bytes(g, la, 0, hi);
            else
                __builtin_nontemporal_store(*reinterpret_cast<u32x4*>(la), reinterpret_cast<u32x4*>(g));
        }
    }
}

template <int FMT, int VARIANT, bool SA, bool SC, int NORM, bool NAT, int THREADS = 256>
__global__ void __launch_bounds__(THREADS)
fwd_tiled_halo(const uint8_t* __restrict__ aos_arg, uint8_t* __restrict__ soa_arg, uint64_t total_blocks, uint64_t first_block,
               Shifts sh_arg)
{
    __shared__ __attribute__((aligned(16))) uint8_t lds[halo_lds_bytes<FMT, THREADS>()];
    WG_MARK(0);
    const uint32_t wg = blockIdx.x;
    const Shifts sh = shifts_fetched_at_once(sh_arg);
    const uint8_t* __restrict__ aos = fetched_now(aos_arg);
    uint8_t* __restrict__ soa = fetched_now(soa_arg);
    const bool whole = wg < sh.full_tiles;
    const uint64_t tile = !whole ? (uint64_t)sh.full_tiles : shifts_xcd_contiguous(sh, false) ? xcd_contiguous_tile(wg, sh.full_tiles) : (uint64_t)wg;
    const bool edge = !whole || tile == 0;
    if (edge)
        fwd_halo_edge_tile<FMT, VARIANT, SA, SC, NORM, NAT, THREADS>(aos, soa, sh, tile, lds);
    else
        fwd_halo_tile<FMT, VARIANT, SA, SC, NORM, NAT, THREADS>(aos, soa, total_blocks, first_block, sh, tile, lds);
}

template <int FMT, bool SA, bool SC, int W, int THREADS = 256>
__device__ __forceinline__ void inv_shift_load_wave(const uint8_t* __restrict__ soa, uint8_t* lds, int t,
                                                    const uint64_t (&gb)[6], const Shifts& sh, uint64_t total_bytes)
{
    constexpr Streams S = make_streams(FMT, SA, SC);
    constexpr int T = tile_blocks(FMT, THREADS);
    constexpr int wave_lo = W * 1024, wave_hi = wave_lo + 1024;
    const int o = t * 16;
    int la = 0, k = 0, shift = 0;
    uint64_t g = 0;
    static_for<0, S.n>([&](auto si) {
        constexpr int s = decltype(si)::value;
        constexpr int lo = S.off[s] * T;
        constexpr int hi = lo + S.width[s] * T;
        if constexpr (lo < wave_hi && hi > wave_lo) {
            constexpr bool only = lo <= wave_lo && hi >= wave_hi;
            if (only || (o >= lo && o < hi)) {
                la = lo + 16 * s + (o - lo);
                g = gb[s] + (uint64_t)(o - lo);
                k = (o - lo) >> 4;
                shift = sh.d[s];
            }
        }
    });
    const bool main_inside = g + 16 <= total_bytes;
    int la_t = 0, shift_t = 0;
    uint64_t g_t = 0;
    bool has_tail = false, tail_inside = false;
    if constexpr (W == 0) {
#pragma unroll
        for (int ss = 0; ss < S.n; ++ss) {
            if (ss == t) {
                const int bytes = S.width[ss] * T;
                la_t = S.off[ss] * T + 16 * ss + bytes;
                shift_t = sh.d[ss];
                g_t = gb[ss] + bytes;
            }
        }
        has_tail = t < S.n && shift_t > 0;
        tail_inside = g_t + 16 <= total_bytes;
    }
    u32x4 v_main = {0, 0, 0, 0}, v_tail = {0, 0, 0, 0};
    int tail_flags = (has_tail ? 1 : 0) | (tail_inside ? 2 : 0);
    asm volatile("" : "+v"(v_main), "+v"(v_tail), "+v"(g_t), "+v"(tail_flags));
    has_tail = (tail_flags & 1) != 0;
    tail_inside = (tail_flags & 2) != 0;
    if (main_inside)
        v_main = gload16(soa + g);
    if constexpr (W == 0) {
        if (has_tail && tail_inside)
            v_tail = gload16(soa + g_t);
        if (has_tail) {
            if (tail_inside)
                lds_at<u32x4>(lds, la_t) = v_tail;
            else
                copy_partial_segment<false>(lds + la_t, soa + g_t, 0, shift_t);
        }
    }
    if (main_inside)
        lds_at<u32x4>(lds, la) = v_main;
    else
        copy_partial_segment<false>(lds + la, soa + g, (k == 0) ? shift : 0, (k == 0) ? 16 : shift);
}

template <int FMT, int VARIANT, bool SA, bool SC, int THREADS = 256, typename SINK = AosSink>
__device__ __forceinline__ void inv_shift_tile(const uint8_t* __restrict__ soa, uint8_t* __restrict__ aos,
                                               uint64_t total_blocks, uint64_t , const Shifts& sh, uint64_t tile,
                                               uint8_t* lds, const SINK& sink = SINK{})
{
    constexpr Streams S = make_streams(FMT, SA, SC);
    constexpr int T = tile_blocks(FMT, THREADS);
    const int t = threadIdx.x;
    int base[6];
#pragma unroll
    for (int s = 0; s < 6; ++s)
        base[s] = s < S.n ? S.off[s] * T + 16 * s + sh.d[s] : 0;

    const uint64_t total_bytes = total_blocks * (uint64_t)fmt_block(FMT);
    uint64_t gb[6];
    slice_bases<FMT, SA, SC, T>(tile, sh, gb);
    if constexpr (THREADS == 256) {
        switch (__builtin_amdgcn_readfirstlane(t >> 6)) {
        case 0: inv_shift_load_wave<FMT, SA, SC, 0>(soa, lds, t, gb, sh, total_bytes); break;
        case 1: inv_shift_load_wave<FMT, SA, SC, 1>(soa, lds, t, gb, sh, total_bytes); break;
        case 2: inv_shift_load_wave<FMT, SA, SC, 2>(soa, lds, t, gb, sh, total_bytes); break;
        default: inv_shift_load_wave<FMT, SA, SC, 3>(soa, lds, t, gb, sh, total_bytes); break;
        }
    } else {
        for_this_wave<THREADS / 64>(t, [&](auto wi) {
            inv_shift_load_wave<FMT, SA, SC, decltype(wi)::value, THREADS>(soa, lds, t, gb, sh, total_bytes);
        });
    }
    __syncthreads();
    const u32x4 q = sh.natural ? gather_shifted<FMT, VARIANT, SA, SC, true>(lds, t, base)
                               : gather_shifted<FMT, VARIANT, SA, SC, false>(lds, t, base);
    sink.template store<FMT, THREADS>(aos, tile, t, q);
}

template <int FMT, int VARIANT, bool SA, bool SC, int THREADS = 256, typename SINK = AosSink>
__device__ __forceinline__ void inv_shift_edge_tile(const uint8_t* __restrict__ soa, uint8_t* __restrict__ aos,
                                                    uint64_t total_blocks, const Shifts& sh, uint64_t tile, uint8_t* lds,
                                                    const SINK& sink = SINK{})
{
    constexpr Streams S = make_streams(FMT, SA, SC);
    constexpr int T = tile_blocks(FMT, THREADS);
    constexpr int PV = 16 / fmt_block(FMT);
    const int t = threadIdx.x;
    int base[6];
#pragma unroll
    for (int s = 0; s < 6; ++s)
        base[s] = s < S.n ? S.off[s] * T + 16 * s + sh.d[s] : 0;
    const uint64_t left = sh.range_blocks - tile * (uint64_t)T;
    const int own = left < (uint64_t)T ? (int)left : T;
    const uint64_t total_bytes = total_blocks * (uint64_t)fmt_block(FMT);
    uint64_t gb[6];
    slice_bases<FMT, SA, SC, T>(tile, sh, gb);
    auto plan = [&](const EdgeSlot& e, int& lo, int& hi, bool& whole) {
        const int vhi = e.d + e.width * own;
        lo = e.d - e.wo > 0 ? e.d - e.wo : 0;
        hi = vhi - e.wo < 16 ? vhi - e.wo : 16;
        const uint64_t g = e.g + (uint64_t)(int64_t)e.wo;
        whole = total_bytes >= 16 && g <= total_bytes - 16;
    };
    const EdgeSlot em = edge_slot_of_image_byte<FMT, SA, SC, T, T, 16, 0>(t * 16, sh, gb);
    const EdgeSlot ex = edge_slot_behind_window<FMT, SA, SC, T, T, 16, 0>(t, 0, sh, gb);
    int mlo, mhi, xlo = 0, xhi = 0;
    bool mwhole, xwhole = false;
    plan(em, mlo, mhi, mwhole);
    if (t < S.n)
        plan(ex, xlo, xhi, xwhole);
    const uint8_t* gm = soa + em.g + (uint64_t)(int64_t)em.wo;
    const uint8_t* gx = soa + ex.g + (uint64_t)(int64_t)ex.wo;
    u32x4 vm = {0u, 0u, 0u, 0u}, vx = {0u, 0u, 0u, 0u};
    if (mhi > mlo && mwhole)
        vm = *reinterpret_cast<const u32x4*>(gm);
    if (xhi > xlo && xwhole)
        vx = *reinterpret_cast<const u32x4*>(gx);
    if (mhi > mlo) {
        if (mwhole)
            *reinterpret_cast<u32x4*>(lds + em.lds_base + em.wo) = vm;
        else
            copy_segment_bytes(lds + em.lds_base + em.wo, gm, mlo, mhi);
    }
    if (xhi > xlo) {
        if (xwhole)
            *reinterpret_cast<u32x4*>(lds + ex.lds_base + ex.wo) = vx;
        else
            copy_segment_bytes(lds + ex.lds_base + ex.wo, gx, xlo, xhi);
    }
    __builtin_amdgcn_s_waitcnt(0x0F70);
    __syncthreads();
    if (t * PV < own) {
        const u32x4 q = sh.natural ? gather_shifted<FMT, VARIANT, SA, SC, true>(lds, t, base)
                                   : gather_shifted<FMT, VARIANT, SA, SC, false>(lds, t, base);
        sink.template store_edge<FMT, THREADS>(aos, tile, t, q, own);
    }
}

template <int FMT, int VARIANT, bool SA, bool SC, int THREADS = 256>
__global__ void __launch_bounds__(THREADS)
inv_tiled_shift(const uint8_t* __restrict__ soa_arg, uint8_t* __restrict__ aos_arg, uint64_t total_blocks, uint64_t first_block,
                Shifts sh_arg)
{
    __shared__ __attribute__((aligned(16))) uint8_t lds[shift_lds_bytes(1, THREADS)];
    const uint32_t wg = blockIdx.x;
    const Shifts sh = shifts_fetched_at_once(sh_arg);
    const uint8_t* __restrict__ soa = fetched_now(soa_arg);
    uint8_t* __restrict__ aos = fetched_now(aos_arg);
    asm("" : "+s"(total_blocks));
    const bool whole = wg < sh.full_tiles;
    const uint64_t tile = !whole ? (uint64_t)sh.full_tiles : shifts_xcd_contiguous(sh, true) ? xcd_contiguous_tile(wg, sh.full_tiles) : (uint64_t)wg;
    const bool edge = !whole;
    if (edge)
        inv_shift_edge_tile<FMT, VARIANT, SA, SC, THREADS>(soa, aos, total_blocks, sh, tile, lds);
    else
        inv_shift_tile<FMT, VARIANT, SA, SC, THREADS>(soa, aos, total_blocks, first_block, sh, tile, lds);
}

template <int W>
__device__ __forceinline__ void store_bytes(uint8_t* p, uint64_t v, bool natural)
{
    if (natural) {
        if constexpr (W == 1) *p = (uint8_t)v;
        if constexpr (W == 2) *reinterpret_cast<uint16_t*>(p) = (uint16_t)v;
        if constexpr (W == 4) *reinterpret_cast<uint32_t*>(p) = (uint32_t)v;
        if constexpr (W == 8) *reinterpret_cast<uint64_t*>(p) = v;
    } else {
#pragma unroll
        for (int i = 0; i < W; ++i)
            p[i] = (uint8_t)(v >> (8 * i));
    }
}

template <int W>
__device__ __forceinline__ uint64_t load_bytes(const uint8_t* p, bool natural)
{
    if (natural) {
        if constexpr (W == 1) return *p;
        if constexpr (W == 2) return *reinterpret_cast<const uint16_t*>(p);
        if constexpr (W == 4) return *reinterpret_cast<const uint32_t*>(p);
        if constexpr (W == 8) return *reinterpret_cast<const uint64_t*>(p);
    }
    uint64_t v = 0;
#pragma unroll
    for (int i = 0; i < W; ++i)
        v |= (uint64_t)p[i] << (8 * i);
    return v;
}

__device__ __forceinline__ bool aligned_to(const void* p, int a) { return (reinterpret_cast<uintptr_t>(p) & (a - 1)) == 0; }


}

#ifdef DXTLT_EXPERIMENTS
#include "bcn_experiments.h"
#endif
```

dxt-lossless-transform_amd/csrc/bcn_launch.h:

```cpp
#pragma once
#include <hip/hip_runtime_api.h>
#include <stddef.h>
#include <stdint.h>

#include <cstdlib>

namespace dxtlt {

inline const char* experiment_env(const char* name)
{
#ifdef DXTLT_EXPERIMENTS
    return std::getenv(name);
#else
    (void)name;
    return nullptr;
#endif
}

enum Format : int { kBc1 = 1, kBc2 = 2, kBc3 = 3, kBc4 = 4, kBc5 = 5 };

struct Settings {
    int variant;
    bool split_alpha;
    bool split_colour;
    int normalize = 0;
};

struct Range {
    uint64_t total_blocks;
    uint64_t first_block;
    uint64_t num_blocks;
};

struct LaunchTuning {
    int tile_threads;
    int force_generic;
    int xcd_remap;
};

int launch_force_mask();

struct DebugPlannedLaunch {
    int32_t kind;
    int32_t threads;
    uint32_t workgroups;
    uint32_t full_tiles;
    uint64_t range_blocks;
    uint64_t aos_offset;
    uint8_t shift[6];
    uint8_t halo_vecs;
    uint8_t natural;
    uint64_t gbase[6];
};
int debug_plan_transform(Format fmt, bool inverse, const Settings& s, uint64_t src_address, uint64_t dst_address, const Range& r,
                         const LaunchTuning* tuning, DebugPlannedLaunch* out, int cap);

hipError_t launch_transform(Format fmt, bool inverse, const Settings& s, const void* src, void* dst,
                            const Range& r, hipStream_t stream, const LaunchTuning* tuning = nullptr);

hipError_t launch_fill_splitmix64(void* dst, size_t len_bytes, uint64_t seed, uint64_t first_qword,
                                  hipStream_t stream);

hipError_t launch_normalize_bc1_blocks(const void* in, void* out, uint64_t num_blocks, int mode, hipStream_t stream);
hipError_t launch_normalize_bc1_split(void* colours, void* indices, uint64_t num_blocks, int mode, hipStream_t stream);
hipError_t launch_normalize_bc1_all_modes(const void* in, void* const out[3], uint64_t num_blocks, uint32_t* d_any,
                                          hipStream_t stream);
hipError_t launch_bc1_any_normalizable(const void* in, uint64_t num_blocks, uint32_t* d_any, hipStream_t stream);

hipError_t launch_decode_blocks(int fmt, const void* in, void* out, uint64_t num_blocks, hipStream_t stream);
hipError_t launch_count_pixel_differences(int fmt, const void* a, const void* b, uint64_t num_blocks, uint64_t* d_count,
                                          hipStream_t stream);

hipError_t launch_color565_ycocg(bool inverse, const void* in, void* out, uint64_t num_items, int variant, hipStream_t stream);
hipError_t launch_color565_recorrelate_split(const void* src0, const void* src1, void* dst, uint64_t num_items, int variant,
                                             hipStream_t stream);
hipError_t launch_split_565_color_endpoints(const void* in, void* out, uint64_t len_bytes, hipStream_t stream);

hipError_t launch_normalize_bc23_blocks(int fmt, const void* in, void* out, uint64_t num_blocks, int alpha_mode, int color_mode,
                                        hipStream_t stream);
hipError_t launch_normalize_bc23_all_modes(int fmt, const void* in, void* const* outs, uint64_t num_blocks, hipStream_t stream);
hipError_t launch_normalize_bc2_split(void* colours, void* indices, uint64_t num_blocks, int color_mode, hipStream_t stream);
hipError_t launch_normalize_bc3_split(void* alpha_endpoints, void* alpha_indices, void* color_endpoints, void* color_indices,
                                      uint64_t num_blocks, int alpha_mode, int color_mode, hipStream_t stream);

struct BatchEntry {
    const uint8_t* src;
    uint8_t* dst;
    uint64_t blocks;
    uint32_t first_wg;
    uint32_t end_wg;
    uint32_t full_tiles;
    uint8_t form;
    uint8_t halo_vecs;
    uint8_t natural;
    uint8_t reserved;
    uint8_t shift[6];
    uint8_t reserved2[2];
    uint64_t gbase[6];
};
static_assert(sizeof(BatchEntry) == 96, "BatchEntry layout is shared between host and device");

constexpr uint32_t kBatchIndexWgs = 64, kBatchBaseWgs = 4096;
inline size_t batch_index_base_count(uint32_t total_wgs) { return ((size_t)total_wgs + kBatchBaseWgs - 1) / kBatchBaseWgs; }
inline size_t batch_index_delta_count(uint32_t total_wgs) { return ((size_t)total_wgs + kBatchIndexWgs - 1) / kBatchIndexWgs; }
inline size_t batch_index_bytes(uint32_t total_wgs)
{
    return (batch_index_base_count(total_wgs) * 4 + 2 * batch_index_delta_count(total_wgs) + 15) & ~(size_t)15;
}

uint32_t plan_batch_entry(Format fmt, bool inverse, const Settings& s, BatchEntry& e);

hipError_t launch_table_upload(const void* host_mapped, void* dev, size_t bytes, hipStream_t stream);

hipError_t launch_batch(Format fmt, bool inverse, const Settings& s, const BatchEntry* d_entries, const uint8_t* d_index,
                        uint32_t n_entries, uint32_t total_wgs, uint32_t uniform_wgs, bool wide_index, hipStream_t stream,
                        const BatchEntry* strided_first = nullptr, int64_t src_stride = 0, int64_t dst_stride = 0);

bool build_batch_index(const BatchEntry* entries, size_t n_entries, uint32_t total_wgs, uint8_t* index);

hipError_t launch_tiled_array(Format fmt, bool inverse, const Settings& s, const void* first_src, void* first_dst,
                              uint64_t blocks, uint32_t n_buffers, int64_t src_stride, int64_t dst_stride, hipStream_t stream);

inline int block_bytes(Format f) { return f == kBc1 || f == kBc4 ? 8 : 16; }

constexpr bool format_has_alpha_split(int fmt) { return fmt == kBc3 || fmt == kBc4 || fmt == kBc5; }
constexpr bool format_has_colour(int fmt) { return fmt == kBc1 || fmt == kBc2 || fmt == kBc3; }
inline Settings effective_settings(Format f, const Settings& s)
{
    Settings e = s;
    e.split_alpha = format_has_alpha_split(f) && s.split_alpha;
    if (!format_has_colour(f)) {
        e.variant = 0;
        e.split_colour = false;
    }
    return e;
}

struct Streams {
    int n;
    int width[6];
    int off[6];
};

constexpr Streams make_streams(int fmt, bool split_alpha, bool split_colour)
{
    Streams s{};
    int n = 0, off = 0;
    if (fmt == kBc4 || fmt == kBc5) {
        for (int h = 0; h < (fmt == kBc5 ? 2 : 1); ++h) {
            if (split_alpha) {
                s.width[n] = 1; s.off[n] = off; off += 1; ++n;
                s.width[n] = 1; s.off[n] = off; off += 1; ++n;
            } else {
                s.width[n] = 2; s.off[n] = off; off += 2; ++n;
            }
            s.width[n] = 6; s.off[n] = off; off += 6; ++n;
        }
        s.n = n;
        return s;
    }
    if (fmt == kBc3) {
        if (split_alpha) {
            s.width[n] = 1; s.off[n] = off; off += 1; ++n;
            s.width[n] = 1; s.off[n] = off; off += 1; ++n;
        } else {
            s.width[n] = 2; s.off[n] = off; off += 2; ++n;
        }
        s.width[n] = 6; s.off[n] = off; off += 6; ++n;
    }
    if (fmt == kBc2) {
        s.width[n] = 8; s.off[n] = off; off += 8; ++n;
    }
    if (split_colour) {
        s.width[n] = 2; s.off[n] = off; off += 2; ++n;
        s.width[n] = 2; s.off[n] = off; off += 2; ++n;
    } else {
        s.width[n] = 4; s.off[n] = off; off += 4; ++n;
    }
    s.width[n] = 4; s.off[n] = off; off += 4; ++n;
    s.n = n;
    return s;
}

}
```

dxt-lossless-transform_amd/csrc/table_ring.h:

```cpp
#pragma once
#include <hip/hip_runtime_api.h>
#include <stddef.h>

namespace dxtlt_host {

constexpr int kTableSlots = 4;

struct TableSlot {
    void* host = nullptr;
    void* host_mapped = nullptr;
    void* dev = nullptr;
    size_t cap = 0;
    hipEvent_t done = nullptr;
    bool pending = false;
};

struct TableRing {
    int device = -1;
    TableSlot slots[kTableSlots];
    int next = 0;

    ~TableRing() { release(); }
    void release()
    {
        if (device < 0)
            return;
        for (auto& s : slots) {
            if (s.host) (void)hipHostFree(s.host);
            if (s.dev) (void)hipFree(s.dev);
            if (s.done) (void)hipEventDestroy(s.done);
            s = TableSlot{};
        }
        device = -1;
        next = 0;
    }
    hipError_t acquire(size_t bytes, TableSlot** out)
    {
        int dev = 0;
        hipError_t e = hipGetDevice(&dev);
        if (e != hipSuccess)
            return e;
        if (dev != device) {
            release();
            device = dev;
        }
        TableSlot& s = slots[next];
        next = (next + 1) % kTableSlots;
        if (s.pending) {
            e = hipEventSynchronize(s.done);
            if (e != hipSuccess)
                return e;
            s.pending = false;
        }
        if (s.done == nullptr) {
            e = hipEventCreateWithFlags(&s.done, hipEventDisableTiming);
            if (e != hipSuccess)
                return e;
        }
        if (s.cap < bytes) {
            if (s.host) (void)hipHostFree(s.host);
            if (s.dev) (void)hipFree(s.dev);
            s.host = s.dev = nullptr;
            s.cap = 0;
            const size_t want = bytes + bytes / 2 + 4096;
            e = hipHostMalloc(&s.host, want, hipHostMallocMapped);
            if (e == hipSuccess)
                e = hipHostGetDevicePointer(&s.host_mapped, s.host, 0);
            if (e == hipSuccess)
                e = hipMalloc(&s.dev, want);
            if (e != hipSuccess)
                return e;
            s.cap = want;
        }
        *out = &s;
        return hipSuccess;
    }
};

TableRing& thread_table_ring();

hipError_t upload_table(TableSlot* slot, size_t bytes, hipStream_t stream);

}
```

include/dxtlt_gfx950.h:

```cpp
#ifndef DXTLT_GFX950_H
#define DXTLT_GFX950_H

#include <stdbool.h>
#include <stddef.h>
#include <stdint.h>

#include "dlt_size_estimator.h"

#ifdef __cplusplus
extern "C" {
#endif

#define DXTLT_OK 0
#define DXTLT_E_INVALID_LENGTH 1
#define DXTLT_E_INVALID_ARGUMENT 2
#define DXTLT_E_NO_DEVICE 3
#define DXTLT_E_DEVICE 4
#define DXTLT_E_ESTIMATOR 5
#define DXTLT_E_ALLOCATION 6

#define DXTLT_YCOCG_NONE 0
#define DXTLT_YCOCG_VARIANT1 1
#define DXTLT_YCOCG_VARIANT2 2
#define DXTLT_YCOCG_VARIANT3 3

int32_t dxtlt_transform_bc1_with_settings(const uint8_t *input_ptr, uint8_t *output_ptr, size_t len,
                                          uint8_t decorrelation_mode, bool split_colour_endpoints);
int32_t dxtlt_untransform_bc1_with_settings(const uint8_t *input_ptr, uint8_t *output_ptr, size_t len,
                                            uint8_t decorrelation_mode, bool split_colour_endpoints);
int32_t dxtlt_transform_bc2_with_settings(const uint8_t *input_ptr, uint8_t *output_ptr, size_t len,
                                          uint8_t decorrelation_mode, bool split_colour_endpoints);
int32_t dxtlt_untransform_bc2_with_settings(const uint8_t *input_ptr, uint8_t *output_ptr, size_t len,
                                            uint8_t decorrelation_mode, bool split_colour_endpoints);
int32_t dxtlt_transform_bc3_with_settings(const uint8_t *input_ptr, uint8_t *output_ptr, size_t len,
                                          uint8_t decorrelation_mode, bool split_alpha_endpoints,
                                          bool split_colour_endpoints);
int32_t dxtlt_untransform_bc3_with_settings(const uint8_t *input_ptr, uint8_t *output_ptr, size_t len,
                                            uint8_t decorrelation_mode, bool split_alpha_endpoints,
                                            bool split_colour_endpoints);

int32_t dxtlt_transform_bc1_auto(const uint8_t *input_ptr, uint8_t *output_ptr, size_t len,
                                 const DltSizeEstimator *estimator, bool use_all_decorrelation_modes,
                                 uint8_t *out_decorrelation_mode, bool *out_split_colour_endpoints,
                                 uint32_t *out_estimator_error);
int32_t dxtlt_transform_bc2_auto(const uint8_t *input_ptr, uint8_t *output_ptr, size_t len,
                                 const DltSizeEstimator *estimator, bool use_all_decorrelation_modes,
                                 uint8_t *out_decorrelation_mode, bool *out_split_colour_endpoints,
                                 uint32_t *out_estimator_error);
int32_t dxtlt_transform_bc3_auto(const uint8_t *input_ptr, uint8_t *output_ptr, size_t len,
                                 const DltSizeEstimator *estimator, bool use_all_decorrelation_modes,
                                 uint8_t *out_decorrelation_mode, bool *out_split_alpha_endpoints,
                                 bool *out_split_colour_endpoints, uint32_t *out_estimator_error);

void dxtlt_set_auto_estimator_threads(int32_t threads);
int32_t dxtlt_get_auto_estimator_threads(void);
int32_t dxtlt_set_auto_estimator_threads_for_this_thread(int32_t cap);

int32_t dxtlt_transform_bc1_with_settings_device(const void *d_input, void *d_output, size_t len,
                                                 uint8_t decorrelation_mode, bool split_colour_endpoints,
                                                 void *hip_stream);
int32_t dxtlt_untransform_bc1_with_settings_device(const void *d_input, void *d_output, size_t len,
                                                   uint8_t decorrelation_mode, bool split_colour_endpoints,
                                                   void *hip_stream);
int32_t dxtlt_transform_bc2_with_settings_device(const void *d_input, void *d_output, size_t len,
                                                 uint8_t decorrelation_mode, bool split_colour_endpoints,
                                                 void *hip_stream);
int32_t dxtlt_untransform_bc2_with_settings_device(const void *d_input, void *d_output, size_t len,
                                                   uint8_t decorrelation_mode, bool split_colour_endpoints,
                                                   void *hip_stream);
int32_t dxtlt_transform_bc3_with_settings_device(const void *d_input, void *d_output, size_t len,
                                                 uint8_t decorrelation_mode, bool split_alpha_endpoints,
                                                 bool split_colour_endpoints, void *hip_stream);
int32_t dxtlt_untransform_bc3_with_settings_device(const void *d_input, void *d_output, size_t len,
                                                   uint8_t decorrelation_mode, bool split_alpha_endpoints,
                                                   bool split_colour_endpoints, void *hip_stream);

int32_t dxtlt_transform_range_device(int32_t format, bool inverse, const void *d_src, void *d_dst,
                                     uint64_t total_blocks, uint64_t first_block, uint64_t num_blocks,
                                     uint8_t decorrelation_mode, bool split_alpha_endpoints,
                                     bool split_colour_endpoints, void *hip_stream);

typedef struct DxtltBatchItem {
    const void *d_input;
    void *d_output;
    uint64_t len;
    uint8_t format;
    uint8_t inverse;
    uint8_t decorrelation_mode;
    uint8_t split_alpha_endpoints;
    uint8_t split_colour_endpoints;
    uint8_t reserved[3];
} DxtltBatchItem;
int32_t dxtlt_transform_batch_device(const DxtltBatchItem *items, size_t count, void *hip_stream);
typedef struct DxtltDebugPlannedEntry {
    uint32_t first_wg, end_wg;
    uint32_t full_tiles;
    uint8_t form;
    uint8_t halo_vecs;
    uint8_t shift[6];
    uint64_t gbase[6];
} DxtltDebugPlannedEntry;
uint32_t dxtlt_debug_plan_batch(int32_t format, int32_t inverse, int32_t variant, int32_t split_alpha, int32_t split_colour,
                                const uint64_t *src_addresses, const uint64_t *dst_addresses, const uint64_t *blocks, size_t count,
                                DxtltDebugPlannedEntry *entries_out, uint8_t *index_out, size_t index_capacity,
                                uint32_t *index_is_wide_out);

typedef struct DxtltDebugPlannedLaunch {
    int32_t kind;
    int32_t threads;
    uint32_t workgroups;
    uint32_t full_tiles;
    uint64_t range_blocks;
    uint64_t aos_offset;
    uint8_t shift[6];
    uint8_t halo_vecs;
    uint8_t natural;
    uint64_t gbase[6];
} DxtltDebugPlannedLaunch;
int32_t dxtlt_debug_plan_transform(int32_t format, int32_t inverse, int32_t variant, int32_t split_alpha, int32_t split_colour,
                                   uint64_t src_address, uint64_t dst_address, uint64_t total_blocks, uint64_t first_block,
                                   uint64_t num_blocks, DxtltDebugPlannedLaunch *out, int32_t cap);

int32_t dxtlt_transform_batch_host(const DxtltBatchItem *items, size_t count);

int32_t dxtlt_transform_sharded(int32_t format, bool inverse, const uint8_t *input_ptr, uint8_t *output_ptr,
                                size_t len, uint8_t decorrelation_mode, bool split_alpha_endpoints,
                                bool split_colour_endpoints, int32_t num_devices);

typedef struct DxtltShardStat {
    int32_t device;
    int32_t cpus_bound;
    uint64_t first_block;
    uint64_t blocks;
    double seconds;
} DxtltShardStat;
int32_t dxtlt_sharded_last_stats(DxtltShardStat *out, int32_t cap);

int32_t dxtlt_pci_local_cpulist(const char *pci_bdf, char *out, size_t cap);
int32_t dxtlt_device_local_cpulist(int32_t device, char *out, size_t cap);
int32_t dxtlt_bind_thread_to_cpulist(const char *cpulist);

int32_t dxtlt_fill_splitmix64_device(void *d_dst, size_t len_bytes, uint64_t seed, uint64_t first_qword,
                                     void *hip_stream);
const char *dxtlt_last_error(void);
int32_t dxtlt_device_count(void);
size_t dxtlt_host_route_threshold_bytes(void);
void dxtlt_set_host_route_threshold_bytes(size_t bytes);
void dxtlt_set_tuning(int32_t tile_threads, int32_t force_path);
int32_t dxtlt_tuning_mask(void);
const char *dxtlt_version(void);
void dxtlt_release_thread_resources(void);

#ifdef __cplusplus
}
#endif
#endif
```

Before: 3186.

## Move batch entry planning to a GPU planner kernel with compact host records

Host-side batch planning now writes compact 32-byte records straight into the pinned table ring instead of building full 96-byte BatchEntry structs and index tables. A new device planner kernel expands those records into full entries and builds the wg-to-entry index on the GPU. Groups whose items share size and stride are detected so the launch can skip the table. This aims to cut host CPU planning and upload bytes per batch, at the cost of an extra kernel launch and more complex planning code.

```diff
diff --git a/dxt-lossless-transform_amd/_build.py b/dxt-lossless-transform_amd/_build.py
--- a/dxt-lossless-transform_amd/_build.py
+++ b/dxt-lossless-transform_amd/_build.py
@@ -11,7 +11,7 @@
 LIB_PATH = os.path.join(_HERE, "libdxtlt_gfx950.so")
 _BUILD_DIR = os.path.join(os.path.dirname(_HERE), "build")
 
-SOURCES = ["bcn_kernels.hip", "batch_kernels.hip", "dxtlt_api.cpp", "host_staging.cpp", "host_sharded.cpp", "c_api_core.cpp", "c_api_stable.cpp", "auto_transform.cpp", "file_format.cpp",
+SOURCES = ["bcn_kernels.hip", "batch_kernels.hip", "batch_plan_kernels.hip", "dxtlt_api.cpp", "host_staging.cpp", "host_sharded.cpp", "c_api_core.cpp", "c_api_stable.cpp", "auto_transform.cpp", "file_format.cpp",
            "bc7_kernels.hip", "bc7_api.cpp", "bc6h_kernels.hip", "bc6h_api.cpp", "granule_launch.cpp", "granule_host.cpp", "bc1_normalize.hip", "normalize_api.cpp", "batch_api.cpp", "bc23_normalize.hip",
            "normalize23_api.cpp", "color565_ops.hip", "color565_api.cpp", "bcn_decode.hip", "decode_api.cpp",
            "auto_kernels.hip", "numa_affinity.cpp", "estimate_kernels.hip", "estimate_api.cpp", "batch_auto_kernels.hip", "batch_auto_api.cpp", "pixel_kernels.hip", "pixels_api.cpp",
diff --git a/dxt-lossless-transform_amd/csrc/batch_api.cpp b/dxt-lossless-transform_amd/csrc/batch_api.cpp
--- a/dxt-lossless-transform_amd/csrc/batch_api.cpp
+++ b/dxt-lossless-transform_amd/csrc/batch_api.cpp
@@ -5,11 +5,13 @@
 #include <cstdlib>
 #include <cstring>
 #include <exception>
+#include <memory>
 #include <mutex>
 #include <thread>
 #include <vector>
 
 #include "../../include/dxtlt_gfx950.h"
+#include "batch_plan.h"
 #include "bcn_launch.h"
 #include "granule_launch.h"
 #include "host_common.h"
@@ -63,110 +65,296 @@
 
 namespace {
 
+using dxtlt::BatchPlanSpan;
+using dxtlt::BatchRecord;
+
+constexpr int kGroups = 5 * 2 * 16;
+inline dxtlt::Settings group_settings(int gi)
+{
+    dxtlt::Settings s{};
+    s.variant = (gi >> 2) & 3;
+    s.split_alpha = ((gi >> 1) & 1) != 0;
+    s.split_colour = (gi & 1) != 0;
+    return s;
+}
+inline dxtlt::Format group_format(int gi) { return (dxtlt::Format)((gi >> 5) + 1); }
+inline bool group_inverse(int gi) { return ((gi >> 4) & 1) != 0; }
+
+constexpr uint32_t kNotTaken = 0xFFFFFFFFu, kLaunchFull = 0xFFFFFFFEu;
+
+struct Group {
+    dxtlt::BatchShape shape;
+    BatchEntry first;
+    uint64_t first_soa = 0;
+    int64_t src_stride = 0, dst_stride = 0;
+    uint32_t n = 0, wgs = 0;
+    uint32_t uniform_wgs = 0;
+    uint32_t largest_delta = 0;
+    bool uniform = true;
+    bool strided = true;
+    bool touched = false;
+    BatchRecord* direct = nullptr;
+    std::vector<BatchRecord> own;
+    std::vector<uint32_t> bases;
+
+    void reset()
+    {
+        if (!touched)
+            return;
+        touched = false;
+        n = wgs = uniform_wgs = largest_delta = 0;
+        uniform = strided = true;
+        src_stride = dst_stride = 0;
+        direct = nullptr;
+        own.clear();
+        bases.clear();
+    }
+    const BatchRecord* records() const { return direct ? direct : own.data(); }
+    bool wide() const { return largest_delta > 255; }
+
+    uint32_t add(const uint8_t* src, uint8_t* dst, uint64_t blocks)
+    {
+        const uint64_t soa = shape.inverse ? (uint64_t)reinterpret_cast<uintptr_t>(src) : (uint64_t)reinterpret_cast<uintptr_t>(dst);
+        touched = true;
+        uint32_t item_wgs;
+        bool like_first;
+        if (n != 0 && blocks == first.blocks && ((soa - first_soa) & 127) == 0) {
+            item_wgs = first.end_wg;
+            like_first = true;
+        } else if (n == 0 || (strided && blocks == first.blocks)) {
+            BatchEntry e{};
+            e.src = src;
+            e.dst = dst;
+            e.blocks = blocks;
+            item_wgs = dxtlt::fill_batch_entry(shape, e);
+            if (item_wgs == kNotTaken)
+                return kNotTaken;
+            if (n == 0) {
+                first = e;
+                first_soa = soa;
+            }
+            like_first = e.form == first.form && std::memcmp(e.shift, first.shift, sizeof e.shift) == 0;
+        } else {
+            item_wgs = dxtlt::batch_item_workgroups(shape, soa, blocks);
+            if (item_wgs == kNotTaken)
+                return kNotTaken;
+            like_first = false;
+        }
+        if ((uint64_t)wgs + item_wgs > 0xFFFFFFull)
+            return kLaunchFull;
+        if (n == 0)
+            uniform_wgs = item_wgs;
+        else if (item_wgs != uniform_wgs)
+            uniform = false;
+        if (n == 1) {
+            src_stride = (int64_t)(src - first.src);
+            dst_stride = (int64_t)(dst - first.dst);
+        }
+        strided = strided && like_first && src == first.src + (int64_t)n * src_stride && dst == first.dst + (int64_t)n * dst_stride;
+        const uint32_t first_wg = wgs, end_wg = wgs + item_wgs;
+        const uint32_t m0 = (first_wg + dxtlt::kBatchIndexWgs - 1) & ~(dxtlt::kBatchIndexWgs - 1);
+        if (m0 < end_wg) {
+            if ((m0 & (dxtlt::kBatchBaseWgs - 1)) != 0)
+                largest_delta = std::max(largest_delta, n - bases.back());
+            for (uint32_t k = (m0 + dxtlt::kBatchBaseWgs - 1) / dxtlt::kBatchBaseWgs; k <= (end_wg - 1) / dxtlt::kBatchBaseWgs; ++k)
+                bases.push_back(n);
+        }
+        const BatchRecord r{src, dst, blocks, first_wg, 0};
+        if (direct)
+            direct[n] = r;
+        else
+            own.push_back(r);
+        wgs = end_wg;
+        ++n;
+        return item_wgs;
+    }
+
+    void append_spans(std::vector<BatchPlanSpan>& out, size_t records_at, size_t entries_at, size_t index_at) const
+    {
+        uint32_t tiles = 0, offs = 0, widths = 0;
+        dxtlt::pack_batch_shape(shape, tiles, offs, widths);
+        const BatchRecord* r = records();
+        for (uint32_t k = 0; k < bases.size(); ++k) {
+            uint32_t hi = n - 1;
+            if (k + 1 < bases.size())
+                hi = r[bases[k + 1]].first_wg == (k + 1) * dxtlt::kBatchBaseWgs ? bases[k + 1] - 1 : bases[k + 1];
+            out.push_back({(uint32_t)records_at, (uint32_t)entries_at, (uint32_t)index_at, bases[k], hi, k, wgs, wide() ? 1u : 0u, tiles, offs, widths, 0});
+        }
+    }
+};
+
+using GranuleEntry = dxtlt::granule::BatchEntry;
+struct GranulePlan {
+    std::vector<GranuleEntry> entries, tails;
+    std::vector<uint32_t> coarse;
+    uint64_t wgs = 0, granules = 0;
+    size_t at = 0, entry_bytes = 0, tail_bytes = 0, bytes = 0;
+    void reset()
+    {
+        entries.clear();
+        tails.clear();
+        coarse.clear();
+        wgs = granules = 0;
+        at = entry_bytes = tail_bytes = bytes = 0;
+    }
+};
+
+struct PlanScratch {
+    Group groups[kGroups];
+    GranulePlan granule_plans[4];
+    std::vector<size_t> singles;
+    std::vector<BatchPlanSpan> spans;
+    size_t last_table_bytes = 0;
+    PlanScratch()
+    {
+        for (int gi = 0; gi < kGroups; ++gi) {
+            groups[gi].shape = dxtlt::batch_shape(group_format(gi), group_inverse(gi), dxtlt::effective_settings(group_format(gi), group_settings(gi)));
+        }
+    }
+    void reset()
+    {
+        for (Group& g : groups)
+            g.reset();
+        for (GranulePlan& p : granule_plans)
+            p.reset();
+        singles.clear();
+        spans.clear();
+    }
+};
+PlanScratch& thread_plan_scratch()
+{
+    thread_local std::unique_ptr<PlanScratch> scratch;
+    if (!scratch)
+        scratch.reset(new PlanScratch);
+    scratch->reset();
+    return *scratch;
+}
+
+inline int group_of(const DxtltBatchItem& it)
+{
+    const bool colour = dxtlt::format_has_colour(it.format);
+    const int sa = dxtlt::format_has_alpha_split(it.format) && it.split_alpha_endpoints ? 1 : 0;
+    const int sc = colour && it.split_colour_endpoints ? 1 : 0, mode = colour ? it.decorrelation_mode : 0;
+    return (((it.format - 1) * 2 + (it.inverse ? 1 : 0)) << 4) | (mode << 2) | (sa << 1) | sc;
+}
+
+inline uint32_t most_span_records(const std::vector<BatchPlanSpan>& spans)
+{
+    uint32_t most = 0;
+    for (const BatchPlanSpan& s : spans)
+        most = std::max(most, s.rec_hi - s.rec_lo + 1);
+    return most;
+}
+
+inline size_t padded16(size_t bytes) { return (bytes + 15) & ~(size_t)15; }
+
+hipError_t upload_range(TableSlot* slot, size_t host_at, size_t dev_at, size_t bytes, hipStream_t stream)
+{
+    if (kTableByCopyEngine)
+        return hipMemcpyAsync(static_cast<uint8_t*>(slot->dev) + dev_at, static_cast<uint8_t*>(slot->host) + host_at, bytes, hipMemcpyHostToDevice, stream);
+    return dxtlt::launch_table_upload(static_cast<uint8_t*>(slot->host_mapped) + host_at, static_cast<uint8_t*>(slot->dev) + dev_at, bytes, stream);
+}
+
+struct Placed {
+    size_t records_at, entries_at, index_at;
+    bool strided;
+};
+
+hipError_t launch_groups(const PlanScratch& plan, const Placed* placed, const TableSlot* slot, hipError_t e, hipStream_t user, bool no_uniform)
+{
+    for (int gi = 0; gi < kGroups && e == hipSuccess; ++gi) {
+        const Group& g = plan.groups[gi];
+        if (g.n == 0)
+            continue;
+        const uint8_t* d = static_cast<const uint8_t*>(slot->dev);
+        const bool strided = placed[gi].strided;
+        e = dxtlt::launch_batch(group_format(gi), group_inverse(gi), group_settings(gi),
+                                reinterpret_cast<const BatchEntry*>(strided ? d : d + placed[gi].entries_at), strided ? d : d + placed[gi].index_at, g.n,
+                                g.wgs, g.uniform && !no_uniform ? g.uniform_wgs : 0, g.wide(), user, strided ? &g.first : nullptr, g.src_stride,
+                                g.dst_stride);
+    }
+    return e;
+}
+
 int32_t batch_device(const DxtltBatchItem* items, size_t count, void* hip_stream, bool pixels_allowed)
 {
     if (count == 0)
         return kOk;
     if (items == nullptr)
         return fail(kInvalidArgument, "NULL item array with count > 0");
+    PlanScratch& plan = thread_plan_scratch();
+    TableSlot* slot = nullptr;
+    int direct_gi = -1;
+    const char* limit = nullptr;
+    const int max_format = pixels_allowed ? 9 : 7;
     for (size_t i = 0; i < count; ++i) {
         const DxtltBatchItem& it = items[i];
-        if (it.format < 1 || it.format > (pixels_allowed ? 9 : 7))
+        if (it.format < 1 || it.format > max_format)
             return fail(kInvalidArgument, kDeviceFormatText);
-        if (it.len % item_block_bytes(it.format) != 0)
+        const unsigned block_shift = it.format == 1 || it.format == 4 ? 3 : 4;
+        if (it.format <= 7 ? (it.len & ((size_t(1) << block_shift) - 1)) != 0 : it.len % item_block_bytes(it.format) != 0)
             return fail(kInvalidLength, "batch item: len is not a multiple of the block size");
         if (it.decorrelation_mode > 3 && dxtlt::format_has_colour(it.format))
             return fail(kInvalidArgument, "batch item: decorrelation_mode must be 0..3");
-        if (it.len > 0 && (it.d_input == nullptr || it.d_output == nullptr))
+        if (it.len == 0)
+            continue;
+        if (it.d_input == nullptr || it.d_output == nullptr)
             return fail(kInvalidArgument, "batch item: NULL device buffer with len > 0");
-        if (pixel_item_overlaps(it))
-            return fail(kInvalidArgument, "batch item: pixel input and output overlap");
-    }
-    for (const int format : {7, 6}) {
-        uint64_t granules[2] = {0, 0};
-        for (size_t i = 0; i < count; ++i)
-            if (items[i].format == format)
-                granules[items[i].inverse ? 1 : 0] += items[i].len / 16 / 1024;
-        if (granules[0] > 0xFFFFFFull || granules[1] > 0xFFFFFFull)
-            return fail(kInvalidArgument, dxtlt::granule::named(format, "batch too large for one launch (256 GiB or more of ", " in one direction)"));
-    }
-    hipStream_t user = static_cast<hipStream_t>(hip_stream);
-
-    struct Group {
-        std::vector<BatchEntry> entries;
-        uint32_t wgs = 0;
-        uint32_t uniform_wgs = 0;
-        bool uniform = true;
-    };
-    constexpr int kGroups = 5 * 2 * 16;
-    std::vector<Group> groups(kGroups);
-    auto group_settings = [](int gi) {
-        dxtlt::Settings s{};
-        s.variant = (gi >> 2) & 3;
-        s.split_alpha = ((gi >> 1) & 1) != 0;
-        s.split_colour = (gi & 1) != 0;
-        return s;
-    };
-    std::vector<size_t> singles;
-    for (size_t i = 0; i < count; ++i) {
-        const DxtltBatchItem& it = items[i];
-        if (it.len == 0 || dxtlt::granule::is_granule_format(it.format) || is_pixel_format(it.format))
-            continue;
-        if (it.len >= (size_t(64) << 30))
-            return fail(kInvalidArgument, "batch item of 64 GiB or more: use the single-buffer entry point");
-        const bool colour = dxtlt::format_has_colour(it.format);
-        const int sa = dxtlt::format_has_alpha_split(it.format) && it.split_alpha_endpoints ? 1 : 0;
-        const int sc = colour && it.split_colour_endpoints ? 1 : 0, mode = colour ? it.decorrelation_mode : 0;
-        const int gi = (((it.format - 1) * 2 + (it.inverse ? 1 : 0)) << 4) | (mode << 2) | (sa << 1) | sc;
-        Group& g = groups[gi];
-        BatchEntry e{};
-        e.src = static_cast<const uint8_t*>(it.d_input);
-        e.dst = static_cast<uint8_t*>(it.d_output);
-        e.blocks = it.len / item_block_bytes(it.format);
-        e.first_wg = g.wgs;
-        const uint32_t wgs = dxtlt::plan_batch_entry((dxtlt::Format)it.format, it.inverse != 0, group_settings(gi), e);
-        if (wgs == 0xFFFFFFFFu) {
-            singles.push_back(i);
-            continue;
-        }
-        if ((uint64_t)g.wgs + wgs > 0xFFFFFFull)
-            return fail(kInvalidArgument, "batch too large for one launch (64 GiB or more of one format, direction and settings)");
-        g.wgs += wgs;
-        g.entries.push_back(e);
-        if (g.entries.size() == 1)
-            g.uniform_wgs = wgs;
-        else if (wgs != g.uniform_wgs)
-            g.uniform = false;
-    }
-    static const bool no_uniform = dxtlt::experiment_env("DXTLT_BATCH_NO_UNIFORM") != nullptr;
-    static const bool no_strided = dxtlt::experiment_env("DXTLT_BATCH_NO_STRIDED") != nullptr;
-
-    using GranuleEntry = dxtlt::granule::BatchEntry;
-    struct GranulePlan {
-        std::vector<GranuleEntry> entries, tails;
-        std::vector<uint32_t> coarse;
-        uint64_t wgs = 0;
-        size_t at = 0, entry_bytes = 0, tail_bytes = 0, bytes = 0;
-    };
-    GranulePlan granule_plans[4];
-    size_t table_bytes = 0;
-    for (int q = 0; q < 4; ++q) {
-        GranulePlan& p = granule_plans[q];
-        const int inverse = q & 1, format = q < 2 ? 7 : 6;
-        for (size_t i = 0; i < count; ++i) {
-            const DxtltBatchItem& it = items[i];
-            if (it.format != format || it.len == 0 || (it.inverse != 0) != (inverse != 0))
+        if (it.format > 5) {
+            if (is_pixel_format(it.format)) {
+                if (pixel_item_overlaps(it))
+                    return fail(kInvalidArgument, "batch item: pixel input and output overlap");
                 continue;
-            const uint64_t blocks = it.len / 16, tail = blocks % 1024, main = blocks - tail;
+            }
+            GranulePlan& p = plan.granule_plans[(it.format == 7 ? 0 : 2) + (it.inverse ? 1 : 0)];
+            const uint64_t blocks = it.len >> block_shift, tail = blocks % 1024, main = blocks - tail;
             const uint8_t* src = static_cast<const uint8_t*>(it.d_input);
             uint8_t* dst = static_cast<uint8_t*>(it.d_output);
+            p.granules += main / 1024;
+            if (p.granules > 0xFFFFFFull)
+                continue;
             if (main != 0) {
                 p.entries.push_back({src, dst, main, (uint32_t)p.wgs, 0});
                 p.wgs += main / 1024;
             }
             if (tail != 0)
                 p.tails.push_back({src + main * 16, dst + main * 16, 0, 0, (uint32_t)tail});
-        }
+            continue;
+        }
+        if (limit != nullptr)
+            continue;
+        if (it.len >= (size_t(64) << 30)) {
+            limit = "batch item of 64 GiB or more: use the single-buffer entry point";
+            continue;
+        }
+        const int gi = group_of(it);
+        Group& g = plan.groups[gi];
+        if (direct_gi < 0) {
+            const hipError_t e = g_ring.acquire(std::max(count * sizeof(BatchRecord) + 4096, plan.last_table_bytes), &slot);
+            if (e != hipSuccess)
+                return fail(kDevice, "batch table staging", e);
+            direct_gi = gi;
+            g.direct = static_cast<BatchRecord*>(slot->host);
+        }
+        const uint32_t wgs = g.add(static_cast<const uint8_t*>(it.d_input), static_cast<uint8_t*>(it.d_output), it.len >> block_shift);
+        if (wgs == kNotTaken)
+            plan.singles.push_back(i);
+        else if (wgs == kLaunchFull)
+            limit = "batch too large for one launch (64 GiB or more of one format, direction and settings)";
+    }
+    for (const int format : {7, 6}) {
+        const GranulePlan* p = &plan.granule_plans[format == 7 ? 0 : 2];
+        if (p[0].granules > 0xFFFFFFull || p[1].granules > 0xFFFFFFull)
+            return fail(kInvalidArgument, dxtlt::granule::named(format, "batch too large for one launch (256 GiB or more of ", " in one direction)"));
+    }
+    if (limit != nullptr)
+        return fail(kInvalidArgument, limit);
+    hipStream_t user = static_cast<hipStream_t>(hip_stream);
+    static const bool no_uniform = dxtlt::experiment_env("DXTLT_BATCH_NO_UNIFORM") != nullptr;
+    static const bool no_strided = dxtlt::experiment_env("DXTLT_BATCH_NO_STRIDED") != nullptr;
+
+    size_t dev_bytes = 0;
+    for (GranulePlan& p : plan.granule_plans) {
         if (p.entries.empty() && p.tails.empty())
             continue;
         p.coarse.resize(((size_t)p.wgs + 63) / 64);
@@ -178,48 +366,70 @@
         }
         p.entry_bytes = p.entries.size() * sizeof(GranuleEntry);
         p.tail_bytes = p.tails.size() * sizeof(GranuleEntry);
-        p.bytes = (p.entry_bytes + p.tail_bytes + p.coarse.size() * sizeof(uint32_t) + 15) & ~(size_t)15;
-        p.at = table_bytes;
-        table_bytes += p.bytes;
-    }
-
-    struct Placed {
-        int gi;
-        size_t at, entry_bytes;
-    };
-    std::vector<Placed> placed;
+        p.bytes = padded16(p.entry_bytes + p.tail_bytes + p.coarse.size() * sizeof(uint32_t));
+        p.at = dev_bytes;
+        dev_bytes += p.bytes;
+    }
+    const size_t granule_bytes = dev_bytes;
+    Placed placed[kGroups] = {};
+    const size_t direct_bytes = direct_gi < 0 ? 0 : plan.groups[direct_gi].n * sizeof(BatchRecord);
+    size_t host_bytes = direct_bytes;
     for (int gi = 0; gi < kGroups; ++gi) {
-        const Group& g = groups[gi];
-        if (g.entries.empty())
+        const Group& g = plan.groups[gi];
+        if (g.n == 0)
             continue;
-        const size_t entry_bytes = (g.entries.size() * sizeof(BatchEntry) + 15) & ~(size_t)15;
-        placed.push_back({gi, table_bytes, entry_bytes});
-        table_bytes += entry_bytes + dxtlt::batch_index_bytes(g.wgs);
-    }
-    if (table_bytes != 0) {
-        TableSlot* slot = nullptr;
-        hipError_t e = g_ring.acquire(table_bytes, &slot);
+        Placed& at = placed[gi];
+        at.strided = g.strided && g.uniform && !no_uniform && !no_strided;
+        if (at.strided)
+            continue;
+        at.records_at = 0;
+        if (gi != direct_gi) {
+            at.records_at = host_bytes;
+            host_bytes += g.n * sizeof(BatchRecord);
+        }
+        at.entries_at = dev_bytes;
+        at.index_at = dev_bytes + padded16(g.n * sizeof(BatchEntry));
+        dev_bytes = at.index_at + dxtlt::batch_index_bytes(g.wgs);
+        g.append_spans(plan.spans, at.records_at, at.entries_at, at.index_at);
+    }
+    const size_t spans_at = host_bytes;
+    host_bytes += plan.spans.size() * sizeof(BatchPlanSpan);
+    const size_t granule_at = host_bytes;
+    host_bytes += granule_bytes;
+    const size_t table_bytes = std::max(host_bytes, dev_bytes);
+    if (granule_bytes != 0 || !plan.spans.empty()) {
+        hipError_t e = hipSuccess;
+        if (table_bytes > (size_t(1) << 31))
+            return fail(kDevice, "batch table copy / launch", hipErrorInvalidValue);
+        if (slot == nullptr)
+            e = g_ring.acquire(table_bytes, &slot);
+        else if (slot->cap < table_bytes)
+            e = g_ring.grow(slot, table_bytes, direct_bytes);
         if (e != hipSuccess)
             return fail(kDevice, "batch table staging", e);
-        for (const GranulePlan& p : granule_plans) {
+        plan.last_table_bytes = table_bytes;
+        uint8_t* host = static_cast<uint8_t*>(slot->host);
+        for (int gi = 0; gi < kGroups; ++gi) {
+            const Group& g = plan.groups[gi];
+            if (g.n != 0 && !placed[gi].strided && gi != direct_gi)
+                std::memcpy(host + placed[gi].records_at, g.own.data(), g.n * sizeof(BatchRecord));
+        }
+        if (!plan.spans.empty())
+            std::memcpy(host + spans_at, plan.spans.data(), plan.spans.size() * sizeof(BatchPlanSpan));
+        for (const GranulePlan& p : plan.granule_plans) {
             if (p.bytes == 0)
                 continue;
-            uint8_t* h = static_cast<uint8_t*>(slot->host) + p.at;
+            uint8_t* h = host + granule_at + p.at;
             if (p.entry_bytes) std::memcpy(h, p.entries.data(), p.entry_bytes);
             if (p.tail_bytes) std::memcpy(h + p.entry_bytes, p.tails.data(), p.tail_bytes);
             if (!p.coarse.empty()) std::memcpy(h + p.entry_bytes + p.tail_bytes, p.coarse.data(), p.coarse.size() * sizeof(uint32_t));
         }
-        std::vector<bool> wide(placed.size());
-        for (size_t k = 0; k < placed.size(); ++k) {
-            const Group& g = groups[placed[k].gi];
-            uint8_t* h = static_cast<uint8_t*>(slot->host) + placed[k].at;
-            std::memcpy(h, g.entries.data(), g.entries.size() * sizeof(BatchEntry));
-            wide[k] = dxtlt::build_batch_index(g.entries.data(), g.entries.size(), g.wgs, h + placed[k].entry_bytes);
-        }
-        e = upload_table(slot, table_bytes, user);
+        e = dxtlt::launch_batch_planner(slot->host_mapped, slot->dev, (uint32_t)spans_at, (uint32_t)plan.spans.size(), most_span_records(plan.spans), user);
+        if (e == hipSuccess && granule_bytes != 0)
+            e = upload_range(slot, granule_at, 0, granule_bytes, user);
         const char* what = "batch table copy / launch";
         for (int q = 0; q < 4 && e == hipSuccess; ++q) {
-            const GranulePlan& p = granule_plans[q];
+            const GranulePlan& p = plan.granule_plans[q];
             const int inverse = q & 1, format = q < 2 ? 7 : 6;
             if (p.bytes == 0)
                 continue;
@@ -231,33 +441,17 @@
             if (e != hipSuccess)
                 what = format == 7 ? "BC7 batch table copy / launch" : "BC6H batch table copy / launch";
         }
-        for (size_t k = 0; k < placed.size() && e == hipSuccess; ++k) {
-            const int gi = placed[k].gi;
-            Group& g = groups[gi];
-            const size_t n = g.entries.size();
-            const bool uniform = g.uniform && !no_uniform;
-            bool strided = uniform && !no_strided;
-            const int64_t src_stride = n >= 2 ? (int64_t)(g.entries[1].src - g.entries[0].src) : 0;
-            const int64_t dst_stride = n >= 2 ? (int64_t)(g.entries[1].dst - g.entries[0].dst) : 0;
-            for (size_t i = 1; i < n && strided; ++i) {
-                const BatchEntry &a = g.entries[0], &b = g.entries[i];
-                strided = b.blocks == a.blocks && b.full_tiles == a.full_tiles && b.form == a.form && b.halo_vecs == a.halo_vecs &&
-                          std::memcmp(b.shift, a.shift, sizeof a.shift) == 0 && std::memcmp(b.gbase, a.gbase, sizeof a.gbase) == 0 &&
-                          b.src == a.src + (int64_t)i * src_stride && b.dst == a.dst + (int64_t)i * dst_stride;
-            }
-            const uint8_t* d = static_cast<const uint8_t*>(slot->dev) + placed[k].at;
-            e = dxtlt::launch_batch((dxtlt::Format)((gi >> 5) + 1), ((gi >> 4) & 1) != 0, group_settings(gi),
-                                    reinterpret_cast<const BatchEntry*>(d), d + placed[k].entry_bytes, (uint32_t)n, g.wgs,
-                                    uniform ? g.uniform_wgs : 0, wide[k], user, strided ? &g.entries[0] : nullptr, src_stride, dst_stride);
-        }
+        e = launch_groups(plan, placed, slot, e, user, no_uniform);
         hipError_t ev = hipEventRecord(slot->done, user);
         slot->pending = ev == hipSuccess;
         if (e != hipSuccess)
             return fail(kDevice, what, e);
         if (ev != hipSuccess)
             return fail(kDevice, "batch event", ev);
-    }
-    for (size_t i : singles) {
+    } else if (hipError_t e = launch_groups(plan, placed, slot, hipSuccess, user, no_uniform); e != hipSuccess) {
+        return fail(kDevice, "batch table copy / launch", e);
+    }
+    for (size_t i : plan.singles) {
         const DxtltBatchItem& it = items[i];
         dxtlt::Settings s{};
         s.variant = it.decorrelation_mode;
@@ -270,10 +464,11 @@
         if (e != hipSuccess)
             return fail(kDevice, "batch item launch", e);
     }
-    for (size_t i = 0; i < count; ++i)
-        if (is_pixel_format(items[i].format) && items[i].len != 0)
-            if (int32_t rc = launch_pixel_item(items[i], user); rc != kOk)
-                return rc;
+    if (pixels_allowed)
+        for (size_t i = 0; i < count; ++i)
+            if (is_pixel_format(items[i].format) && items[i].len != 0)
+                if (int32_t rc = launch_pixel_item(items[i], user); rc != kOk)
+                    return rc;
     return kOk;
 }
 
@@ -335,6 +530,112 @@
 
 namespace {
 
+bool debug_host_pass(int32_t format, int32_t inverse, int32_t variant, int32_t split_alpha, int32_t split_colour, const uint64_t* src_addresses,
+                     const uint64_t* dst_addresses, const uint64_t* blocks, size_t count, Group& g, int& gi, std::vector<uint32_t>& singles)
+{
+    if (format < 1 || format > 5 || variant < 0 || variant > 3 || count > 0xFFFFFFFFull || (count != 0 && (!src_addresses || !dst_addresses || !blocks)))
+        return false;
+    DxtltBatchItem it{};
+    it.format = (uint8_t)format;
+    it.inverse = inverse != 0;
+    it.decorrelation_mode = (uint8_t)variant;
+    it.split_alpha_endpoints = split_alpha != 0;
+    it.split_colour_endpoints = split_colour != 0;
+    gi = group_of(it);
+    g.shape = dxtlt::batch_shape(group_format(gi), inverse != 0, dxtlt::effective_settings(group_format(gi), group_settings(gi)));
+    for (size_t i = 0; i < count; ++i) {
+        if (blocks[i] == 0)
+            continue;
+        const uint32_t wgs = g.add(reinterpret_cast<const uint8_t*>(static_cast<uintptr_t>(src_addresses[i])),
+                                   reinterpret_cast<uint8_t*>(static_cast<uintptr_t>(dst_addresses[i])), blocks[i]);
+        if (wgs == kLaunchFull)
+            return false;
+        if (wgs == kNotTaken)
+            singles.push_back((uint32_t)i);
+    }
+    return true;
+}
+
+void debug_summary(const Group& g, size_t singles, DxtltDebugCompactPlan* out)
+{
+    if (out == nullptr)
+        return;
+    *out = DxtltDebugCompactPlan{};
+    out->records = g.n;
+    out->singles = (uint32_t)singles;
+    out->total_wgs = g.wgs;
+    out->uniform_wgs = g.n != 0 && g.uniform ? g.uniform_wgs : 0;
+    out->is_regular_array = g.n != 0 && g.uniform && g.strided ? 1 : 0;
+    out->index_is_wide = g.wide() ? 1 : 0;
+    out->src_stride = g.src_stride;
+    out->dst_stride = g.dst_stride;
+}
+
+}
+
+extern "C" int32_t dxtlt_debug_plan_batch_compact(int32_t format, int32_t inverse, int32_t variant, int32_t split_alpha, int32_t split_colour,
+                                                  const uint64_t* src_addresses, const uint64_t* dst_addresses, const uint64_t* blocks,
+                                                  size_t count, DxtltDebugBatchRecord* records_out, uint32_t* singles_out,
+                                                  DxtltDebugCompactPlan* summary_out)
+{
+    static_assert(sizeof(DxtltDebugBatchRecord) == sizeof(BatchRecord), "the hook hands the records out as they are staged");
+    Group g;
+    int gi = 0;
+    std::vector<uint32_t> singles;
+    if ((count != 0 && (!records_out || !singles_out)) ||
+        !debug_host_pass(format, inverse, variant, split_alpha, split_colour, src_addresses, dst_addresses, blocks, count, g, gi, singles))
+        return fail(kInvalidArgument, "dxtlt_debug_plan_batch_compact: bad arguments, or a launch of 2^24 workgroups or more");
+    if (g.n != 0)
+        std::memcpy(records_out, g.own.data(), g.n * sizeof(BatchRecord));
+    if (!singles.empty())
+        std::memcpy(singles_out, singles.data(), singles.size() * sizeof(uint32_t));
+    debug_summary(g, singles.size(), summary_out);
+    return kOk;
+}
+
+extern "C" int32_t dxtlt_debug_run_batch_planner(int32_t format, int32_t inverse, int32_t variant, int32_t split_alpha, int32_t split_colour,
+                                                 const uint64_t* src_addresses, const uint64_t* dst_addresses, const uint64_t* blocks,
+                                                 size_t count, uint8_t* entries_out, size_t entries_capacity, uint8_t* index_out,
+                                                 size_t index_capacity, DxtltDebugCompactPlan* summary_out)
+{
+    Group g;
+    int gi = 0;
+    std::vector<uint32_t> singles;
+    if (!debug_host_pass(format, inverse, variant, split_alpha, split_colour, src_addresses, dst_addresses, blocks, count, g, gi, singles) ||
+        !singles.empty())
+        return fail(kInvalidArgument, "dxtlt_debug_run_batch_planner: bad arguments, a buffer the batch kernel does not take, or a launch of 2^24 workgroups or more");
+    debug_summary(g, 0, summary_out);
+    if (g.n == 0)
+        return kOk;
+    const size_t entry_bytes = g.n * sizeof(BatchEntry), index_bytes = dxtlt::batch_index_bytes(g.wgs);
+    if (!entries_out || !index_out || entries_capacity < g.n || index_capacity < index_bytes)
+        return fail(kInvalidArgument, "dxtlt_debug_run_batch_planner: entries_capacity or index_capacity too small");
+    const size_t record_bytes = g.n * sizeof(BatchRecord), index_at = padded16(entry_bytes);
+    std::vector<BatchPlanSpan> spans;
+    g.append_spans(spans, 0, 0, index_at);
+    const size_t table_bytes = std::max(record_bytes + spans.size() * sizeof(BatchPlanSpan), index_at + index_bytes);
+    if (table_bytes > (size_t(1) << 31))
+        return fail(kInvalidArgument, "dxtlt_debug_run_batch_planner: table too large");
+    TableSlot* slot = nullptr;
+    hipError_t e = g_ring.acquire(table_bytes, &slot);
+    if (e != hipSuccess)
+        return fail(kDevice, "batch table staging", e);
+    std::memcpy(slot->host, g.own.data(), record_bytes);
+    std::memcpy(static_cast<uint8_t*>(slot->host) + record_bytes, spans.data(), spans.size() * sizeof(BatchPlanSpan));
+    e = dxtlt::launch_batch_planner(slot->host_mapped, slot->dev, (uint32_t)record_bytes, (uint32_t)spans.size(), most_span_records(spans), nullptr);
+    if (e == hipSuccess)
+        e = hipStreamSynchronize(nullptr);
+    if (e == hipSuccess)
+        e = hipMemcpy(entries_out, slot->dev, entry_bytes, hipMemcpyDeviceToHost);
+    if (e == hipSuccess)
+        e = hipMemcpy(index_out, static_cast<const uint8_t*>(slot->dev) + index_at, index_bytes, hipMemcpyDeviceToHost);
+    if (e != hipSuccess)
+        return fail(kDevice, "batch planner", e);
+    return kOk;
+}
+
+namespace {
+
 size_t env_number(const char* name, size_t fallback)
 {
     const char* v = std::getenv(name);
diff --git a/dxt-lossless-transform_amd/csrc/batch_kernels.hip b/dxt-lossless-transform_amd/csrc/batch_kernels.hip
--- a/dxt-lossless-transform_amd/csrc/batch_kernels.hip
+++ b/dxt-lossless-transform_amd/csrc/batch_kernels.hip
@@ -5,6 +5,7 @@
 #include "bcn_device.h"
 
 #include "batch_lookup.h"
+#include "batch_plan.h"
 
 namespace dxtlt {
 
@@ -186,40 +187,20 @@
 
 uint32_t plan_batch_entry(Format fmt, bool inverse, const Settings& s, BatchEntry& e)
 {
-    if (e.blocks == 0)
-        return 0;
-    const Settings es = effective_settings(fmt, s);
-    const Streams S = make_streams(fmt, es.split_alpha, es.split_colour);
-    const void* soa = inverse ? (const void*)e.src : (const void*)e.dst;
-    const uint64_t T = (uint64_t)tile_blocks(fmt, batch_tile_threads(fmt, es.split_colour, inverse));
-    const uint64_t tiles = e.blocks / T, rest = e.blocks % T;
-    const uint64_t mask = inverse ? 15 : (uint64_t)(kHaloAlign - 1);
-    bool on_lines = true, stream_tails = false;
-    int d[6] = {0, 0, 0, 0, 0, 0}, halo_blocks = 0;
-    for (int i = 0; i < S.n; ++i) {
-        const uint64_t base = reinterpret_cast<uintptr_t>(soa) + (uint64_t)S.off[i] * e.blocks;
-        d[i] = (int)(base & mask);
-        on_lines = on_lines && (base & 127) == 0;
-        stream_tails = stream_tails || d[i] != 0;
-        halo_blocks = std::max(halo_blocks, (d[i] + S.width[i] - 1) / S.width[i]);
-    }
-    if (!shifts_are_natural(S, d))
-        return 0xFFFFFFFFu;
-    e.form = on_lines ? 1 : 0;
-    e.natural = 1;
-    e.reserved = 0;
-    e.reserved2[0] = e.reserved2[1] = 0;
-    const int per_vec = 16 / fmt_block(fmt);
-    e.halo_vecs = inverse ? 0 : (uint8_t)((halo_blocks + per_vec - 1) / per_vec);
-    for (int i = 0; i < 6; ++i) {
-        e.shift[i] = (uint8_t)d[i];
-        e.gbase[i] = i < S.n ? (uint64_t)S.off[i] * e.blocks - (uint64_t)d[i] : 0;
-    }
-    e.full_tiles = (uint32_t)tiles;
-    const bool edge = rest != 0 || (!inverse && stream_tails);
-    const uint32_t wgs = (uint32_t)tiles + (edge ? 1u : 0u);
-    e.end_wg = e.first_wg + wgs;
-    return wgs;
+    return fill_batch_entry(batch_shape(fmt, inverse, effective_settings(fmt, s)), e);
+}
+
+BatchShape batch_shape(Format fmt, bool inverse, const Settings& es)
+{
+    BatchShape g{};
+    g.S = make_streams(fmt, es.split_alpha, es.split_colour);
+    const uint32_t T = (uint32_t)tile_blocks(fmt, batch_tile_threads(fmt, es.split_colour, inverse));
+    while ((1u << g.tile_shift) < T)
+        ++g.tile_shift;
+    g.mask = inverse ? 15u : (uint32_t)(kHaloAlign - 1);
+    g.per_vec = 16u / (uint32_t)fmt_block(fmt);
+    g.inverse = inverse ? 1u : 0u;
+    return g;
 }
 
 bool build_batch_index(const BatchEntry* entries, size_t n_entries, uint32_t total_wgs, uint8_t* index)
diff --git a/dxt-lossless-transform_amd/csrc/batch_plan.h b/dxt-lossless-transform_amd/csrc/batch_plan.h
--- /dev/null
+++ b/dxt-lossless-transform_amd/csrc/batch_plan.h
@@ -0,0 +1,122 @@
+#pragma once
+#include "bcn_launch.h"
+
+#if defined(__HIPCC__) || defined(__HIP__)
+#define DXTLT_PLAN_HD __host__ __device__
+#else
+#define DXTLT_PLAN_HD
+#endif
+
+namespace dxtlt {
+
+struct BatchRecord {
+    const uint8_t* src;
+    uint8_t* dst;
+    uint64_t blocks;
+    uint32_t first_wg;
+    uint32_t reserved;
+};
+static_assert(sizeof(BatchRecord) == 32, "BatchRecord layout is shared between host and device");
+
+struct BatchShape {
+    Streams S;
+    uint32_t tile_shift;
+    uint32_t mask;
+    uint32_t per_vec;
+    uint32_t inverse;
+};
+BatchShape batch_shape(Format fmt, bool inverse, const Settings& effective);
+
+inline void pack_batch_shape(const BatchShape& g, uint32_t& tiles, uint32_t& offs, uint32_t& widths)
+{
+    tiles = g.tile_shift | (g.mask << 8) | (g.per_vec << 16) | (g.inverse << 24);
+    offs = (uint32_t)g.S.n << 24;
+    widths = 0;
+    for (int i = 0; i < g.S.n; ++i) {
+        offs |= (uint32_t)g.S.off[i] << (4 * i);
+        widths |= (uint32_t)g.S.width[i] << (4 * i);
+    }
+}
+DXTLT_PLAN_HD inline BatchShape unpack_batch_shape(uint32_t tiles, uint32_t offs, uint32_t widths)
+{
+    BatchShape g{};
+    g.S.n = (int)(offs >> 24);
+#pragma unroll
+    for (int i = 0; i < 6; ++i) {
+        g.S.off[i] = (int)((offs >> (4 * i)) & 15u);
+        g.S.width[i] = (int)((widths >> (4 * i)) & 15u);
+    }
+    g.tile_shift = tiles & 0xFFu;
+    g.mask = (tiles >> 8) & 0xFFu;
+    g.per_vec = (tiles >> 16) & 0xFFu;
+    g.inverse = tiles >> 24;
+    return g;
+}
+
+DXTLT_PLAN_HD inline uint32_t batch_item_workgroups(const BatchShape& g, uint64_t soa, uint64_t blocks)
+{
+    uint32_t any = 0, odd = 0;
+#pragma unroll
+    for (int i = 0; i < 6; ++i) {
+        if (i < g.S.n) {
+            const uint32_t d = (uint32_t)(soa + (uint64_t)g.S.off[i] * blocks) & g.mask;
+            any |= d;
+            odd |= d & (uint32_t)(stream_element_width(g.S.width[i]) - 1);
+        }
+    }
+    if (odd != 0)
+        return 0xFFFFFFFFu;
+    const uint64_t tiles = blocks >> g.tile_shift, rest = blocks & ((1ull << g.tile_shift) - 1);
+    return (uint32_t)tiles + (rest != 0 || (g.inverse == 0 && any != 0) ? 1u : 0u);
+}
+
+DXTLT_PLAN_HD inline uint32_t fill_batch_entry(const BatchShape& g, BatchEntry& e)
+{
+    if (e.blocks == 0)
+        return 0;
+    const uint64_t soa = g.inverse ? (uint64_t)reinterpret_cast<uintptr_t>(e.src) : (uint64_t)reinterpret_cast<uintptr_t>(e.dst);
+    const uint32_t wgs = batch_item_workgroups(g, soa, e.blocks);
+    if (wgs == 0xFFFFFFFFu)
+        return wgs;
+    bool on_lines = true;
+    uint32_t halo_blocks = 0;
+#pragma unroll
+    for (int i = 0; i < 6; ++i) {
+        uint32_t d = 0;
+        if (i < g.S.n) {
+            const uint64_t base = soa + (uint64_t)g.S.off[i] * e.blocks;
+            d = (uint32_t)base & g.mask;
+            on_lines = on_lines && (base & 127) == 0;
+            const uint32_t in_blocks = (d + (uint32_t)g.S.width[i] - 1) / (uint32_t)g.S.width[i];
+            halo_blocks = halo_blocks > in_blocks ? halo_blocks : in_blocks;
+        }
+        e.shift[i] = (uint8_t)d;
+        e.gbase[i] = i < g.S.n ? (uint64_t)g.S.off[i] * e.blocks - (uint64_t)d : 0;
+    }
+    e.form = on_lines ? 1 : 0;
+    e.natural = 1;
+    e.reserved = 0;
+    e.reserved2[0] = e.reserved2[1] = 0;
+    e.halo_vecs = g.inverse ? 0 : (uint8_t)((halo_blocks + g.per_vec - 1) / g.per_vec);
+    e.full_tiles = (uint32_t)(e.blocks >> g.tile_shift);
+    e.end_wg = e.first_wg + wgs;
+    return wgs;
+}
+
+struct BatchPlanSpan {
+    uint32_t records_at;
+    uint32_t entries_at;
+    uint32_t index_at;
+    uint32_t rec_lo, rec_hi;
+    uint32_t span;
+    uint32_t total_wgs;
+    uint32_t wide;
+    uint32_t tiles, stream_offs, stream_widths;
+    uint32_t reserved;
+};
+static_assert(sizeof(BatchPlanSpan) == 48, "BatchPlanSpan layout is shared between host and device");
+
+hipError_t launch_batch_planner(const void* host_mapped, void* dev, uint32_t spans_at, uint32_t spans, uint32_t most_records,
+                                hipStream_t stream);
+
+}
diff --git a/dxt-lossless-transform_amd/csrc/batch_plan_kernels.hip b/dxt-lossless-transform_amd/csrc/batch_plan_kernels.hip
--- /dev/null
+++ b/dxt-lossless-transform_amd/csrc/batch_plan_kernels.hip
@@ -0,0 +1,93 @@
+#include "batch_plan.h"
+#include "bcn_device.h"
+
+namespace dxtlt {
+
+static_assert(offsetof(BatchEntry, first_wg) == 24 && offsetof(BatchEntry, full_tiles) == 32 && offsetof(BatchEntry, form) == 36 && offsetof(BatchEntry, halo_vecs) == 37 &&
+                  offsetof(BatchEntry, natural) == 38 && offsetof(BatchEntry, shift) == 40 && offsetof(BatchEntry, gbase) == 48,
+              "batch_plan_kernel writes BatchEntry by dword offsets");
+
+namespace {
+
+constexpr int kPlanThreadsDense = 1024, kPlanThreadsSparse = 256;
+constexpr uint32_t kSpanRecords = kBatchBaseWgs + 1;
+
+template <int kPlanThreads>
+__global__ void __launch_bounds__(kPlanThreads)
+batch_plan_kernel(const uint8_t* __restrict__ host, uint8_t* __restrict__ dev, uint32_t spans_at)
+{
+    __shared__ uint32_t first_wg[kSpanRecords];
+    const BatchPlanSpan sp = reinterpret_cast<const BatchPlanSpan*>(host + spans_at)[blockIdx.x];
+    const bool wide = sp.wide != 0;
+    const BatchShape shape = unpack_batch_shape(sp.tiles, sp.stream_offs, sp.stream_widths);
+    const BatchRecord* records = reinterpret_cast<const BatchRecord*>(host + sp.records_at);
+    BatchEntry* entries = reinterpret_cast<BatchEntry*>(dev + sp.entries_at);
+    const uint32_t n = sp.rec_hi - sp.rec_lo + 1u;
+    const uint32_t span_first = sp.span * kBatchBaseWgs;
+    for (uint32_t i = threadIdx.x; i < n && i < kSpanRecords; i += kPlanThreads) {
+        const u32x4* rec = reinterpret_cast<const u32x4*>(&records[sp.rec_lo + i]);
+        const u32x4 lo = rec[0], hi = rec[1];
+        const uint32_t first = hi.z;
+        first_wg[i] = first;
+        if (first < span_first)
+            continue;
+        BatchEntry e;
+        e.src = reinterpret_cast<const uint8_t*>((uintptr_t)(lo.x | ((uint64_t)lo.y << 32)));
+        e.dst = reinterpret_cast<uint8_t*>((uintptr_t)(lo.z | ((uint64_t)lo.w << 32)));
+        e.blocks = hi.x | ((uint64_t)hi.y << 32);
+        e.first_wg = first;
+        (void)fill_batch_entry(shape, e);
+        u32x4* out = reinterpret_cast<u32x4*>(&entries[sp.rec_lo + i]);
+        out[0] = lo;
+        out[1] = u32x4{hi.x, hi.y, first, e.end_wg};
+        out[2] = u32x4{e.full_tiles, (uint32_t)e.form | ((uint32_t)e.halo_vecs << 8) | ((uint32_t)e.natural << 16),
+                       (uint32_t)e.shift[0] | ((uint32_t)e.shift[1] << 8) | ((uint32_t)e.shift[2] << 16) | ((uint32_t)e.shift[3] << 24),
+                       (uint32_t)e.shift[4] | ((uint32_t)e.shift[5] << 8)};
+#pragma unroll
+        for (int k = 0; k < 3; ++k)
+            out[3 + k] = u32x4{(uint32_t)e.gbase[2 * k], (uint32_t)(e.gbase[2 * k] >> 32), (uint32_t)e.gbase[2 * k + 1], (uint32_t)(e.gbase[2 * k + 1] >> 32)};
+    }
+    __syncthreads();
+    const uint32_t n_base = (uint32_t)batch_index_base_count(sp.total_wgs), n_delta = (uint32_t)batch_index_delta_count(sp.total_wgs);
+    uint8_t* index = dev + sp.index_at;
+    if (threadIdx.x == 0)
+        reinterpret_cast<uint32_t*>(index)[sp.span] = sp.rec_lo;
+    uint8_t* delta = index + n_base * 4u;
+    const uint32_t j = sp.span * (kBatchBaseWgs / kBatchIndexWgs) + threadIdx.x;
+    if (threadIdx.x < kBatchBaseWgs / kBatchIndexWgs && j < n_delta) {
+        const uint32_t wg = j * kBatchIndexWgs;
+        uint32_t lo = 0, hi = (n < kSpanRecords ? n : kSpanRecords) - 1u;
+        while (lo < hi) {
+            const uint32_t mid = (lo + hi + 1u) >> 1;
+            if (first_wg[mid] <= wg)
+                lo = mid;
+            else
+                hi = mid - 1u;
+        }
+        if (wide)
+            reinterpret_cast<uint16_t*>(delta)[j] = (uint16_t)lo;
+        else
+            delta[j] = (uint8_t)lo;
+    }
+    const uint32_t used = n_base * 4u + (wide ? 2u : 1u) * n_delta, bytes = (uint32_t)batch_index_bytes(sp.total_wgs);
+    const uint32_t at = used + sp.span * 80u + threadIdx.x;
+    if (threadIdx.x < 80u && at < bytes)
+        index[at] = 0;
+}
+
+}
+
+hipError_t launch_batch_planner(const void* host_mapped, void* dev, uint32_t spans_at, uint32_t spans, uint32_t most_records, hipStream_t stream)
+{
+    if (spans == 0)
+        return hipSuccess;
+    if (most_records > (uint32_t)kPlanThreadsSparse)
+        hipLaunchKernelGGL(batch_plan_kernel<kPlanThreadsDense>, dim3(spans), dim3(kPlanThreadsDense), 0, stream,
+                           static_cast<const uint8_t*>(host_mapped), static_cast<uint8_t*>(dev), spans_at);
+    else
+        hipLaunchKernelGGL(batch_plan_kernel<kPlanThreadsSparse>, dim3(spans), dim3(kPlanThreadsSparse), 0, stream,
+                           static_cast<const uint8_t*>(host_mapped), static_cast<uint8_t*>(dev), spans_at);
+    return hipGetLastError();
+}
+
+}
diff --git a/dxt-lossless-transform_amd/csrc/bcn_device.h b/dxt-lossless-transform_amd/csrc/bcn_device.h
--- a/dxt-lossless-transform_amd/csrc/bcn_device.h
+++ b/dxt-lossless-transform_amd/csrc/bcn_device.h
@@ -544,8 +544,6 @@
 #endif
     return s;
 }
-
-__host__ __device__ constexpr int stream_element_width(int bytes_per_block) { return bytes_per_block == 6 ? 2 : bytes_per_block; }
 
 template <typename STREAMS>
 __host__ __device__ inline int shifts_are_natural(const STREAMS& S, const int (&d)[6])
diff --git a/dxt-lossless-transform_amd/csrc/bcn_launch.h b/dxt-lossless-transform_amd/csrc/bcn_launch.h
--- a/dxt-lossless-transform_amd/csrc/bcn_launch.h
+++ b/dxt-lossless-transform_amd/csrc/bcn_launch.h
@@ -101,9 +101,9 @@
 static_assert(sizeof(BatchEntry) == 96, "BatchEntry layout is shared between host and device");
 
 constexpr uint32_t kBatchIndexWgs = 64, kBatchBaseWgs = 4096;
-inline size_t batch_index_base_count(uint32_t total_wgs) { return ((size_t)total_wgs + kBatchBaseWgs - 1) / kBatchBaseWgs; }
-inline size_t batch_index_delta_count(uint32_t total_wgs) { return ((size_t)total_wgs + kBatchIndexWgs - 1) / kBatchIndexWgs; }
-inline size_t batch_index_bytes(uint32_t total_wgs)
+constexpr size_t batch_index_base_count(uint32_t total_wgs) { return ((size_t)total_wgs + kBatchBaseWgs - 1) / kBatchBaseWgs; }
+constexpr size_t batch_index_delta_count(uint32_t total_wgs) { return ((size_t)total_wgs + kBatchIndexWgs - 1) / kBatchIndexWgs; }
+constexpr size_t batch_index_bytes(uint32_t total_wgs)
 {
     return (batch_index_base_count(total_wgs) * 4 + 2 * batch_index_delta_count(total_wgs) + 15) & ~(size_t)15;
 }
@@ -182,4 +182,6 @@
     return s;
 }
 
+constexpr int stream_element_width(int bytes_per_block) { return bytes_per_block == 6 ? 2 : bytes_per_block; }
+
 }
diff --git a/dxt-lossless-transform_amd/csrc/table_ring.h b/dxt-lossless-transform_amd/csrc/table_ring.h
--- a/dxt-lossless-transform_amd/csrc/table_ring.h
+++ b/dxt-lossless-transform_amd/csrc/table_ring.h
@@ -1,6 +1,7 @@
 #pragma once
 #include <hip/hip_runtime_api.h>
 #include <stddef.h>
+#include <string.h>
 
 namespace dxtlt_host {
 
@@ -75,6 +76,32 @@
         *out = &s;
         return hipSuccess;
     }
+    hipError_t grow(TableSlot* s, size_t bytes, size_t keep)
+    {
+        if (s->cap >= bytes)
+            return hipSuccess;
+        TableSlot bigger;
+        const size_t want = bytes + bytes / 2 + 4096;
+        hipError_t e = hipHostMalloc(&bigger.host, want, hipHostMallocMapped);
+        if (e == hipSuccess)
+            e = hipHostGetDevicePointer(&bigger.host_mapped, bigger.host, 0);
+        if (e == hipSuccess)
+            e = hipMalloc(&bigger.dev, want);
+        if (e != hipSuccess) {
+            if (bigger.host) (void)hipHostFree(bigger.host);
+            if (bigger.dev) (void)hipFree(bigger.dev);
+            return e;
+        }
+        if (keep)
+            memcpy(bigger.host, s->host, keep);
+        if (s->host) (void)hipHostFree(s->host);
+        if (s->dev) (void)hipFree(s->dev);
+        s->host = bigger.host;
+        s->host_mapped = bigger.host_mapped;
+        s->dev = bigger.dev;
+        s->cap = want;
+        return hipSuccess;
+    }
 };
 
 TableRing& thread_table_ring();
diff --git a/include/dxtlt_gfx950.h b/include/dxtlt_gfx950.h
--- a/include/dxtlt_gfx950.h
+++ b/include/dxtlt_gfx950.h
@@ -104,6 +104,21 @@
                                 const uint64_t *src_addresses, const uint64_t *dst_addresses, const uint64_t *blocks, size_t count,
                                 DxtltDebugPlannedEntry *entries_out, uint8_t *index_out, size_t index_capacity,
                                 uint32_t *index_is_wide_out);
+typedef struct DxtltDebugBatchRecord {
+    uint64_t src_address, dst_address, blocks;
+    uint32_t first_wg, reserved;
+} DxtltDebugBatchRecord;
+typedef struct DxtltDebugCompactPlan {
+    uint32_t records, singles, total_wgs, uniform_wgs, is_regular_array, index_is_wide;
+    int64_t src_stride, dst_stride;
+} DxtltDebugCompactPlan;
+int32_t dxtlt_debug_plan_batch_compact(int32_t format, int32_t inverse, int32_t variant, int32_t split_alpha, int32_t split_colour,
+                                       const uint64_t *src_addresses, const uint64_t *dst_addresses, const uint64_t *blocks, size_t count,
+                                       DxtltDebugBatchRecord *records_out, uint32_t *singles_out, DxtltDebugCompactPlan *summary_out);
+int32_t dxtlt_debug_run_batch_planner(int32_t format, int32_t inverse, int32_t variant, int32_t split_alpha, int32_t split_colour,
+                                      const uint64_t *src_addresses, const uint64_t *dst_addresses, const uint64_t *blocks, size_t count,
+                                      uint8_t *entries_out, size_t entries_capacity, uint8_t *index_out, size_t index_capacity,
+                                      DxtltDebugCompactPlan *summary_out);
 
 typedef struct DxtltDebugPlannedLaunch {
     int32_t kind;
```

Result: no change. 3187 (median of 4 runs) (+0.0%).
